# MPEGGroup/mpeg-pcc-tmc2

Measured on AMD Instinct MI355X. Metric: encoder patch+image-gen frames/sec, longdress_vox10 32-frame GOF, higher is better.
Workload: dtype int32/f64

## Files before the change

### mpeg-pcc-tmc2_amd/csrc/api.cpp

```cpp
#include <algorithm>
#include <cstring>
#include <atomic>
#include <chrono>
#include <condition_variable>
#include <cstdarg>
#include <map>
#include <memory>
#include <mutex>

#include "internal.h"

extern char** environ;

namespace tmc2 {
int allowLargeLds( const void* kernel, size_t bytes, int device, size_t staticBytes ) {
  static std::mutex                                 lock;
  static std::map<std::pair<const void*, int>, int> granted;
  std::lock_guard<std::mutex>                       g( lock );
  int& have = granted[{kernel, device}];
  if ( int( bytes ) <= have ) return TMC2_OK;
  const int want = 160 * 1024 - int( ( staticBytes + 63 ) & ~size_t( 63 ) );
  if ( int( bytes ) > want ) {
    setError( "%zu bytes of dynamic LDS requested (+ %zu static): more than a gfx950 workgroup has", bytes, staticBytes );
    return TMC2_E_INVALID;
  }
  TMC2_HIP( hipFuncSetAttribute( kernel, hipFuncAttributeMaxDynamicSharedMemorySize, want ) );
  have = want;
  return TMC2_OK;
}
}

namespace tmc2 {

static thread_local std::string g_lastError;

void setError( const char* fmt, ... ) {
  char    buf[1024];
  va_list ap;
  va_start( ap, fmt );
  vsnprintf( buf, sizeof( buf ), fmt, ap );
  va_end( ap );
  g_lastError = buf;
}

}
struct tmc2_host_gate {
  std::mutex              lock;
  std::condition_variable freed;
  int                     limit = 0, busy = 0;
};
namespace tmc2 {
static std::shared_ptr<tmc2_host_gate> defaultGate() {
  static std::shared_ptr<tmc2_host_gate> g = std::make_shared<tmc2_host_gate>();
  return g;
}
void setHostParallelism( int n ) {
  const auto                  g = defaultGate();
  std::lock_guard<std::mutex> lk( g->lock );
  g->limit = n < 0 ? 0 : n;
  g->freed.notify_all();
}
HostGate::HostGate( const tmc2_ctx* ctx, bool wait ) {
  {
    std::shared_ptr<tmc2_host_gate> own;
    if ( ctx ) {
      std::lock_guard<std::mutex> lk( ctx->optionsLock );
      own = ctx->hostGate;
    }
    gate = own ? own : defaultGate();
  }
  std::unique_lock<std::mutex> lk( gate->lock );
  if ( !wait && gate->limit != 0 && gate->busy >= gate->limit ) return;
  gate->freed.wait( lk, [this] { return gate->limit == 0 || gate->busy < gate->limit; } );
  ++gate->busy;
  held = true;
}
HostGate::~HostGate() { release(); }
void HostGate::release() {
  if ( !held ) return;
  held = false;
  std::lock_guard<std::mutex> g( gate->lock );
  --gate->busy;
  gate->freed.notify_one();
}

static thread_local tmc2_ctx* g_tlsCtx = nullptr;
DevicePool* currentPool() { return g_tlsCtx ? &g_tlsCtx->pool : nullptr; }
ApiScope::ApiScope( tmc2_ctx* ctx ) : prev( g_tlsCtx ) {
  g_tlsCtx = ctx;
  if ( ctx ) (void)hipSetDevice( ctx->device );
}
ApiScope::~ApiScope() { g_tlsCtx = prev; }

int DevicePool::acquire( size_t bytes, void** out, size_t* got ) {
  if ( bytes > ( size_t( 1 ) << 40 ) ) {
    setError( "device allocation of %zu bytes refused", bytes );
    return TMC2_E_INVALID;
  }
  const size_t cls = sizeClass( bytes );
  {
    std::lock_guard<std::mutex> g( lock );
    auto                        it = freeBlocks.find( cls );
    if ( it != freeBlocks.end() && !it->second.empty() ) {
      *out = it->second.back();
      it->second.pop_back();
      *got = cls;
      return TMC2_OK;
    }
  }
  {
    std::lock_guard<std::mutex> g( lock );
    for ( Slab& sl : slabs ) {
      if ( sl.size - sl.used >= cls ) {
        *out = sl.base + sl.used;
        *got = cls;
        sl.used += cls;
        ++carved;
        return TMC2_OK;
      }
    }
  }
  void*      p  = nullptr;
  const auto t0 = std::chrono::steady_clock::now();
  TMC2_HIP( hipMalloc( &p, cls ) );
  const auto t1 = std::chrono::steady_clock::now();
  {
    std::lock_guard<std::mutex> g( lock );
    bytesHeld += cls;
    ++mallocCalls;
    mallocMs += std::chrono::duration<double, std::milli>( t1 - t0 ).count();
  }
  *out = p;
  *got = cls;
  return TMC2_OK;
}
int DevicePool::reserve( size_t bytes ) {
  bytes = ( bytes + 255 ) & ~size_t( 255 );
  void* p = nullptr;
  TMC2_HIP( hipMalloc( &p, bytes ) );
  std::lock_guard<std::mutex> g( lock );
  slabs.push_back( Slab{static_cast<char*>( p ), bytes, 0} );
  bytesHeld += bytes;
  return TMC2_OK;
}
void DevicePool::recycle( void* p, size_t cls ) {
  std::lock_guard<std::mutex> g( lock );
  freeBlocks[cls].push_back( p );
}
void DevicePool::drain() {
  std::lock_guard<std::mutex> g( lock );
  const auto inSlab = [&]( const void* p ) {
    for ( const Slab& sl : slabs )
      if ( static_cast<const char*>( p ) >= sl.base && static_cast<const char*>( p ) < sl.base + sl.size ) return true;
    return false;
  };
  for ( auto& kv : freeBlocks )
    for ( void* p : kv.second )
      if ( !inSlab( p ) ) (void)hipFree( p );
  freeBlocks.clear();
  for ( const Slab& sl : slabs ) (void)hipFree( sl.base );
  slabs.clear();
}

void orientNormalsSpanningTree( const int16_t* xyz, size_t n, const uint32_t* knn, int k, double* normals, void* scratch );

}

using namespace tmc2;

int tmc2_ctx::stageBegin( const char* name ) {
  int id = -1;
  for ( size_t i = 0; i < stages.size(); ++i )
    if ( stages[i].name == name ) id = int( i );
  if ( id < 0 ) {
    StageTimer t;
    t.name = name;
    stages.push_back( t );
    id = int( stages.size() ) - 1;
  }
  stages[id].calls++;
  if ( !timing ) return id;
  hipEvent_t e0 = nullptr, e1 = nullptr;
  if ( freeEvents.size() >= 2 ) {
    e0 = freeEvents.back();
    freeEvents.pop_back();
    e1 = freeEvents.back();
    freeEvents.pop_back();
  } else {
    (void)hipEventCreate( &e0 );
    (void)hipEventCreate( &e1 );
  }
  (void)hipEventRecord( e0, stream );
  stages[id].pending.emplace_back( e0, e1 );
  return id;
}
void tmc2_ctx::stageEnd( int id ) {
  if ( id < 0 || !timing || stages[id].pending.empty() ) return;
  (void)hipEventRecord( stages[id].pending.back().second, stream );
}
void tmc2_ctx::foldStage( StageTimer& t ) {
  for ( auto& pr : t.pending ) {
    float ms = 0.f;
    if ( hipEventSynchronize( pr.second ) == hipSuccess && hipEventElapsedTime( &ms, pr.first, pr.second ) == hipSuccess )
      t.ms += ms;
    freeEvents.push_back( pr.first );
    freeEvents.push_back( pr.second );
  }
  t.pending.clear();
}
void tmc2_ctx::stageAddHostMs( const char* name, double ms ) {
  for ( auto& s : stages )
    if ( s.name == name ) {
      s.ms += ms;
      s.calls++;
      return;
    }
  StageTimer t;
  t.name  = name;
  t.ms    = ms;
  t.calls = 1;
  stages.push_back( t );
}

extern "C" {

const char* tmc2_last_error( void ) { return g_lastError.c_str(); }

int tmc2_ctx_create( int device, tmc2_ctx** out ) {
  if ( !out ) return TMC2_E_INVALID;
  *out      = nullptr;
  int count = 0;
  if ( hipGetDeviceCount( &count ) != hipSuccess || count <= 0 ) {
    setError( "no HIP device visible: this library has no CPU path" );
    return TMC2_E_NO_DEVICE;
  }
  if ( device < 0 || device >= count ) {
    setError( "device %d out of range (%d visible)", device, count );
    return TMC2_E_INVALID;
  }
  TMC2_HIP( hipSetDevice( device ) );
  tmc2_ctx* c = new tmc2_ctx();
  c->device   = device;
  hipDeviceProp_t prop;
  if ( hipGetDeviceProperties( &prop, device ) == hipSuccess ) c->cuCount = prop.multiProcessorCount;
  for ( char** e = environ; e && *e; ++e ) {
    if ( strncmp( *e, "TMC2_", 5 ) != 0 ) continue;
    const char* eq = strchr( *e, '=' );
    if ( !eq ) continue;
    c->options[std::string( *e + 5, size_t( eq - ( *e + 5 ) ) )] = std::string( eq + 1 );
  }
  if ( hipStreamCreateWithFlags( &c->stream, hipStreamNonBlocking ) != hipSuccess ) {
    setError( "hipStreamCreate failed" );
    delete c;
    return TMC2_E_HIP;
  }
  if ( hipHostMalloc( reinterpret_cast<void**>( &c->mailbox ), tmc2_ctx::kMailboxWords * 4, hipHostMallocDefault ) != hipSuccess ) {
    setError( "hipHostMalloc failed (the context's mailbox)" );
    (void)hipStreamDestroy( c->stream );
    delete c;
    return TMC2_E_HIP;
  }
  memset( c->mailbox, 0, tmc2_ctx::kMailboxWords * 4 );
  *out = c;
  return TMC2_OK;
}

int tmc2_ctx_set_option( tmc2_ctx* ctx, const char* key, const char* value ) {
  if ( !ctx || !key || !*key ) {
    tmc2::setError( "tmc2_ctx_set_option: invalid argument" );
    return TMC2_E_INVALID;
  }
  const std::string k = strncmp( key, "TMC2_", 5 ) == 0 ? key + 5 : key;
  std::lock_guard<std::mutex> g( ctx->optionsLock );
  if ( value )
    ctx->options[k] = value;
  else
    ctx->options.erase( k );
  return TMC2_OK;
}
const char* tmc2_ctx_get_option( tmc2_ctx* ctx, const char* key ) {
  if ( !ctx || !key ) return nullptr;
  const auto v = tmc2::ctxOption( ctx, strncmp( key, "TMC2_", 5 ) == 0 ? key + 5 : key );
  if ( !v ) return nullptr;
  static thread_local std::string held;
  held = *v;
  return held.c_str();
}

int tmc2_ctx_reserve( tmc2_ctx* ctx, uint64_t maxPoints, int voxelDimRefine, int bits3d, int maxCanvasWidth, int maxCanvasHeight ) {
  if ( !ctx || maxPoints == 0 || maxPoints > ( uint64_t( 1 ) << 32 ) || bits3d < 1 || bits3d > 16 || maxCanvasWidth < 0 || maxCanvasHeight < 0 ) {
    tmc2::setError( "tmc2_ctx_reserve: invalid argument" );
    return TMC2_E_INVALID;
  }
  tmc2::ApiScope scope( ctx );
  const uint64_t perPoint = voxelDimRefine > 0 && voxelDimRefine <= 2 ? 5500 : 2400;
  const int      gridShift = std::max( 1, bits3d - 1 - ( voxelDimRefine >= 4 ? 2 : ( voxelDimRefine >= 2 ? 1 : 0 ) ) );
  const uint64_t dense     = ( uint64_t( 1 ) << std::min( 33, 3 * gridShift + 1 ) ) / 32 * 8;
  const uint64_t bytes     = maxPoints * perPoint + uint64_t( maxCanvasWidth ) * uint64_t( maxCanvasHeight ) * 64 + dense + ( uint64_t( 64 ) << 20 );
  if ( !ctx->hostC.get<uint32_t>( 4 + ( size_t( maxPoints ) + 4 ) / 4 + 4 ) || !ctx->hostA.get<tmc2::OrientClusterRec>( 64 * 1024 ) ||
       !ctx->hostE.get<tmc2::OrientCompactEdge>( 384 * 1024 ) ) {
    tmc2::setError( "tmc2_ctx_reserve: hipHostMalloc failed" );
    return TMC2_E_HIP;
  }
  return ctx->pool.reserve( size_t( bytes ) );
}
int tmc2_ctx_pool_stats( tmc2_ctx* ctx, uint64_t* bytesHeld, uint64_t* mallocCalls, double* mallocMs, uint64_t* carvedBlocks ) {
  if ( !ctx ) return TMC2_E_INVALID;
  std::lock_guard<std::mutex> g( ctx->pool.lock );
  if ( bytesHeld ) *bytesHeld = ctx->pool.bytesHeld;
  if ( mallocCalls ) *mallocCalls = ctx->pool.mallocCalls;
  if ( mallocMs ) *mallocMs = ctx->pool.mallocMs;
  if ( carvedBlocks ) *carvedBlocks = ctx->pool.carved;
  return TMC2_OK;
}

int tmc2_ctx_device_alloc( tmc2_ctx* ctx, size_t bytes, void** out ) {
  if ( !ctx || !out ) return TMC2_E_INVALID;
  tmc2::ApiScope scope( ctx );
  *out = nullptr;
  TMC2_HIP( hipMalloc( out, std::max<size_t>( bytes, 1 ) ) );
  return TMC2_OK;
}
int tmc2_ctx_device_free( tmc2_ctx* ctx, void* p ) {
  if ( !ctx ) return TMC2_E_INVALID;
  tmc2::ApiScope scope( ctx );
  if ( p ) TMC2_HIP( hipFree( p ) );
  return TMC2_OK;
}
int tmc2_ctx_upload( tmc2_ctx* ctx, void* deviceDst, const void* hostSrc, size_t bytes ) {
  if ( !ctx || ( bytes && ( !deviceDst || !hostSrc ) ) ) return TMC2_E_INVALID;
  tmc2::ApiScope scope( ctx );
  if ( bytes ) TMC2_HIP( hipMemcpyAsync( deviceDst, hostSrc, bytes, hipMemcpyHostToDevice, ctx->stream ) );
  return TMC2_OK;
}
int tmc2_ctx_download( tmc2_ctx* ctx, void* hostDst, const void* deviceSrc, size_t bytes ) {
  if ( !ctx || ( bytes && ( !hostDst || !deviceSrc ) ) ) return TMC2_E_INVALID;
  tmc2::ApiScope scope( ctx );
  if ( bytes ) TMC2_HIP( hipMemcpyAsync( hostDst, deviceSrc, bytes, hipMemcpyDeviceToHost, ctx->stream ) );
  TMC2_HIP( hipStreamSynchronize( ctx->stream ) );
  return TMC2_OK;
}
void* tmc2_ctx_stream( tmc2_ctx* ctx ) { return ctx ? static_cast<void*>( ctx->stream ) : nullptr; }
int   tmc2_ctx_device( tmc2_ctx* ctx ) { return ctx ? ctx->device : -1; }
int   tmc2_ctx_make_current( tmc2_ctx* ctx ) {
  if ( !ctx ) return TMC2_E_INVALID;
  TMC2_HIP( hipSetDevice( ctx->device ) );
  return TMC2_OK;
}

void tmc2_ctx_destroy( tmc2_ctx* ctx ) {
  if ( !ctx ) return;
  ctx->destroyRequested.store( true );
  if ( ctx->liveFrames.load() > 0 ) return;
  if ( ctx->destroyClaimed.exchange( true ) ) return;
  tmc2::destroyContextNow( ctx );
}
}

void tmc2::destroyContextNow( tmc2_ctx* ctx ) {
  (void)hipSetDevice( ctx->device );
  for ( auto& s : ctx->stages ) ctx->foldStage( s );
  for ( auto e : ctx->freeEvents ) (void)hipEventDestroy( e );
  {
    ApiScope scope( ctx );
    ctx->gridBits.release();
    ctx->scanState.release();
    ctx->voxelBitmap.release();
    ctx->constTables.clear();
    ctx->retiredTables.clear();
  }
  if ( ctx->stream ) (void)hipStreamSynchronize( ctx->stream );
  ctx->pool.drain();
  if ( ctx->stream ) (void)hipStreamDestroy( ctx->stream );
  if ( ctx->mailbox ) (void)hipHostFree( ctx->mailbox );
  delete ctx;
}

extern "C" {

int tmc2_host_alloc( size_t bytes, void** out ) {
  if ( !out || bytes == 0 ) return TMC2_E_INVALID;
  *out = nullptr;
  if ( hipHostMalloc( out, bytes, hipHostMallocPortable ) != hipSuccess ) {
    (void)hipGetLastError();
    setError( "host_alloc: %zu bytes of page-locked memory refused", bytes );
    return TMC2_E_HIP;
  }
  return TMC2_OK;
}
void tmc2_host_free( void* p ) {
  if ( p ) (void)hipHostFree( p );
}
int tmc2_host_register( void* p, size_t bytes ) {
  if ( !p || bytes == 0 ) return TMC2_E_INVALID;
  if ( hipHostRegister( p, bytes, hipHostRegisterPortable ) != hipSuccess ) {
    (void)hipGetLastError();
    setError( "host_register: %zu bytes at %p could not be page-locked", bytes, p );
    return TMC2_E_HIP;
  }
  return TMC2_OK;
}
int tmc2_host_unregister( void* p ) {
  if ( !p ) return TMC2_E_INVALID;
  if ( hipHostUnregister( p ) != hipSuccess ) {
    (void)hipGetLastError();
    return TMC2_E_HIP;
  }
  return TMC2_OK;
}

void tmc2_set_host_parallelism( int maxConcurrentHostSteps ) { tmc2::setHostParallelism( maxConcurrentHostSteps ); }
namespace {
std::mutex                                                  g_gatesLock;
std::map<tmc2_host_gate*, std::shared_ptr<tmc2_host_gate>> g_gates;
}
int tmc2_host_gate_create( int maxConcurrentHostSteps, tmc2_host_gate** out ) {
  if ( !out || maxConcurrentHostSteps < 0 ) {
    tmc2::setError( "tmc2_host_gate_create: invalid argument" );
    return TMC2_E_INVALID;
  }
  auto g   = std::make_shared<tmc2_host_gate>();
  g->limit = maxConcurrentHostSteps;
  std::lock_guard<std::mutex> lk( g_gatesLock );
  g_gates[g.get()] = g;
  *out             = g.get();
  return TMC2_OK;
}
void tmc2_host_gate_destroy( tmc2_host_gate* gate ) {
  std::lock_guard<std::mutex> lk( g_gatesLock );
  g_gates.erase( gate );
}
int tmc2_ctx_set_host_gate( tmc2_ctx* ctx, tmc2_host_gate* gate ) {
  if ( !ctx ) {
    tmc2::setError( "tmc2_ctx_set_host_gate: invalid argument" );
    return TMC2_E_INVALID;
  }
  std::shared_ptr<tmc2_host_gate> g;
  if ( gate ) {
    std::lock_guard<std::mutex> lk( g_gatesLock );
    const auto                  it = g_gates.find( gate );
    if ( it == g_gates.end() ) {
      tmc2::setError( "tmc2_ctx_set_host_gate: not a live gate" );
      return TMC2_E_INVALID;
    }
    g = it->second;
  }
  std::lock_guard<std::mutex> lk( ctx->optionsLock );
  ctx->hostGate = g;
  return TMC2_OK;
}

int tmc2_ctx_synchronize( tmc2_ctx* ctx ) {
  if ( !ctx ) return TMC2_E_INVALID;
  TMC2_HIP( hipStreamSynchronize( ctx->stream ) );
  return TMC2_OK;
}

int tmc2_ctx_stage_count( tmc2_ctx* ctx ) { return ctx ? int( ctx->stages.size() ) : 0; }
const char* tmc2_ctx_stage_name( tmc2_ctx* ctx, int i ) {
  return ( ctx && i >= 0 && i < int( ctx->stages.size() ) ) ? ctx->stages[i].name.c_str() : "";
}
double tmc2_ctx_stage_ms( tmc2_ctx* ctx, int i ) {
  if ( !ctx || i < 0 || i >= int( ctx->stages.size() ) ) return 0.0;
  auto& s = ctx->stages[i];
  ctx->foldStage( s );
  return s.ms;
}
void tmc2_ctx_stage_reset( tmc2_ctx* ctx ) {
  if ( !ctx ) return;
  for ( auto& s : ctx->stages ) {
    ctx->foldStage( s );
    s.ms    = 0.0;
    s.calls = 0;
  }
}
long tmc2_ctx_stage_calls( tmc2_ctx* ctx, int i ) {
  return ( ctx && i >= 0 && i < int( ctx->stages.size() ) ) ? ctx->stages[i].calls : 0;
}
void tmc2_ctx_set_timing( tmc2_ctx* ctx, int enabled ) {
  if ( ctx ) ctx->timing = enabled != 0;
}

int tmc2_frame_create( tmc2_ctx* ctx, const int16_t* xyz, const uint8_t* rgb, uint64_t n, tmc2_frame** out ) {
  if ( !ctx || !xyz || !out || n == 0 || n > 0x7FFFFFF0ull ) {
    setError( "frame_create: invalid argument" );
    return TMC2_E_INVALID;
  }
  *out = nullptr;
  ApiScope                    scope( ctx );
  std::unique_ptr<tmc2_frame> f( new tmc2_frame() );
  f->ticket.bind( ctx );
  f->ctx = ctx;
  f->n   = n;
  f->h_xyz.assign( xyz, xyz + 3 * n );
  for ( uint64_t i = 0; i < 3 * n; ++i ) f->geoMax = std::max( f->geoMax, xyz[i] );
  if ( rgb ) f->h_rgb.assign( rgb, rgb + 3 * n );
  std::vector<Pt> pts( n );
  for ( uint64_t i = 0; i < n; ++i ) pts[i] = Pt{xyz[3 * i], xyz[3 * i + 1], xyz[3 * i + 2], 0};
  TMC2_TRY( f->d_pts.alloc( n ) );
  hipStream_t s = ctx->stream;
  TMC2_HIP( hipMemcpyAsync( f->d_pts.p, pts.data(), n * sizeof( Pt ), hipMemcpyHostToDevice, s ) );
  TMC2_HIP( hipStreamSynchronize( s ) );
  if ( rgb ) {
    std::vector<uint8_t> c4( n * 4 );
    for ( uint64_t i = 0; i < n; ++i ) {
      c4[4 * i]     = rgb[3 * i];
      c4[4 * i + 1] = rgb[3 * i + 1];
      c4[4 * i + 2] = rgb[3 * i + 2];
      c4[4 * i + 3] = 0;
    }
    TMC2_TRY( f->d_rgb.alloc( n * 4 ) );
    TMC2_HIP( hipMemcpyAsync( f->d_rgb.p, c4.data(), n * 4, hipMemcpyHostToDevice, s ) );
    TMC2_HIP( hipStreamSynchronize( s ) );
  }
  TMC2_HIP( hipStreamSynchronize( s ) );
  *out = f.release();
  return TMC2_OK;
}

}

namespace tmc2 {
std::optional<std::string> ctxOption( const tmc2_ctx* ctx, const char* key ) {
  if ( !ctx ) {
    const std::string name = std::string( "TMC2_" ) + key;
    const char*       e    = getenv( name.c_str() );
    return e ? std::optional<std::string>( e ) : std::nullopt;
  }
  std::lock_guard<std::mutex> g( ctx->optionsLock );
  const auto                  it = ctx->options.find( key );
  if ( it == ctx->options.end() ) return std::nullopt;
  return it->second;
}
static std::atomic<int> g_refineOverlap{-1};
bool refineOverlap( const tmc2_ctx* ctx ) {
  if ( const auto e = ctxOption( ctx, "REFINE_OVERLAP" ) ) return ( *e )[0] == '1';
  return g_refineOverlap.load( std::memory_order_relaxed ) > 0;
}
static std::atomic<int> g_kdtreeOnHost{-1};
int kdtreePlacement( const tmc2_ctx* ctx ) {
  if ( const auto e = ctxOption( ctx, "KDTREE_HOST" ) )
    if ( ( *e )[0] >= '0' && ( *e )[0] <= '2' ) return ( *e )[0] - '0';
  const int v = g_kdtreeOnHost.load( std::memory_order_relaxed );
  return v < 0 ? 0 : v;
}
int unionPrecheck( const tmc2_ctx* ctx ) {
  const auto e = ctxOption( ctx, "UF_PRECHECK" );
  return e ? ( ( *e )[0] != '0' ) : 1;
}
bool unionAgentScope( const tmc2_ctx* ctx ) {
  const auto e = ctxOption( ctx, "UF_SCOPE" );
  return e && ( *e )[0] == 'a';
}
bool unionCheck( const tmc2_ctx* ctx ) {
  const auto e = ctxOption( ctx, "UF_CHECK" );
  return e && ( *e )[0] == '1';
}
int unionCheckResult( hipStream_t s, const uint32_t* d_bad, const std::string& what ) {
  uint32_t bad[2] = {0, 0};
  TMC2_HIP( hipMemcpyAsync( bad, d_bad, 8, hipMemcpyDeviceToHost, s ) );
  TMC2_HIP( hipStreamSynchronize( s ) );
  if ( bad[0] | bad[1] ) {
    setError( "%s (%u bad links, %u split edges)", what.c_str(), bad[0], bad[1] );
    return TMC2_E_HIP;
  }
  return TMC2_OK;
}
PassOrder passOrder( const tmc2_frame* f, const char* option ) {
  const auto order = ctxOption( f->ctx, option );
  const char o     = order ? ( *order )[0] : 'c';
  const bool tree  = o == 't' && f->haveTree && f->tree.perm.p && f->tree.perm.count >= f->n;
  return {o != 'i', tree ? f->tree.perm.p : nullptr};
}
void setRefineOverlapDefault( int on ) { g_refineOverlap.store( on ? 1 : 0, std::memory_order_relaxed ); }
void setKdtreePlacement( int mode ) { g_kdtreeOnHost.store( mode < 0 || mode > 2 ? 0 : mode, std::memory_order_relaxed ); }
int buildKdTreePlaced( tmc2_ctx* ctx, const Pt* d_pts, uint64_t n, const int16_t* hostXyz, const char* stage, DeviceTree& tree ) {
  const int placement = kdtreePlacement( ctx );
  HostGate gate( ctx, placement == 1 );
  if ( placement == 0 || !gate.held ) {
    StageScope span( ctx, stage );
    return buildKdTreeDevice( ctx, d_pts, n, tree );
  }
  Pt*       hp = ctx->hostD.get<Pt>( n );
  uint32_t* hi = ctx->hostA.get<uint32_t>( n );
  if ( !hp || !hi ) {
    setError( "kdtree: hipHostMalloc failed" );
    return TMC2_E_HIP;
  }
  hipStream_t s = ctx->stream;
  if ( !hostXyz ) {
    TMC2_HIP( hipMemcpyAsync( hp, d_pts, n * sizeof( Pt ), hipMemcpyDeviceToHost, s ) );
    TMC2_HIP( hipStreamSynchronize( s ) );
  }
  KdTreeHost host;
  {
    const auto t0 = std::chrono::steady_clock::now();
    if ( hostXyz )
      for ( uint64_t i = 0; i < n; ++i ) hp[i] = Pt{hostXyz[3 * size_t( i )], hostXyz[3 * size_t( i ) + 1], hostXyz[3 * size_t( i ) + 2], 0};
    host.buildInPlace( hp, hi, n );
    const auto t1 = std::chrono::steady_clock::now();
    ctx->stageAddHostMs( ( std::string( stage ) + "_host" ).c_str(), std::chrono::duration<double, std::milli>( t1 - t0 ).count() );
  }
  gate.release();
  TMC2_TRY( tree.ptsTree.alloc( n ) );
  TMC2_TRY( tree.perm.alloc( n ) );
  TMC2_TRY( tree.nodes.alloc( host.nodes.size() ) );
  TMC2_HIP( hipMemcpyAsync( tree.ptsTree.p, hp, n * sizeof( Pt ), hipMemcpyHostToDevice, s ) );
  TMC2_HIP( hipMemcpyAsync( tree.perm.p, hi, n * sizeof( uint32_t ), hipMemcpyHostToDevice, s ) );
  TMC2_HIP( hipMemcpyAsync( tree.nodes.p, host.nodes.data(), host.nodes.size() * sizeof( KdNode ), hipMemcpyHostToDevice, s ) );
  TMC2_HIP( hipStreamSynchronize( s ) );
  for ( int d = 0; d < 3; ++d ) tree.lo[d] = host.lo[d], tree.hi[d] = host.hi[d];
  tree.depth = host.depth;
  tree.n     = n;
  return TMC2_OK;
}
}

const int* tmc2_ctx::constTable( uint64_t key, const std::vector<int>& host ) {
  auto it = constTables.find( key );
  if ( it != constTables.end() && it->second->host == host ) return it->second->dev.p;
  auto entry = std::make_unique<ConstTable>();
  if ( entry->dev.alloc( std::max<size_t>( host.size(), 1 ) ) != TMC2_OK ) return nullptr;
  entry->host = host;
  if ( !host.empty() && hipMemcpyAsync( entry->dev.p, entry->host.data(), host.size() * sizeof( int ), hipMemcpyHostToDevice, stream ) != hipSuccess ) {
    tmc2::setError( "constTable: upload failed" );
    return nullptr;
  }
  const int* p = entry->dev.p;
  if ( it != constTables.end() ) retiredTables.push_back( std::move( it->second ) );
  constTables[key] = std::move( entry );
  return p;
}

void tmc2_frame::resetDerived() {
  haveTree = haveKnn = haveNormals = havePartition = haveMutual = false;
  havePatches = haveAttr16 = false;
  patchesChanged();
  patches.clear();
  packOrder.clear();
  packMatch.clear();
  depthCount = occCount = 0;
  rounds = packedHeight = packedWidth = 0;
  refineJob.reset();
}

int tmc2::normalsCompute( tmc2_frame* f, int k, int orientation, const std::function<int()>* beforeHostWalk ) {
  TMC2_TRY( tmc2_normals_compute_normals( f, k ) );
  if ( orientation == 0 ) return TMC2_OK;
  if ( orientation != 1 ) {
    setError( "normalOrientation=%d unsupported (0 none, 1 spanning tree)", orientation );
    return TMC2_E_UNSUPPORTED;
  }
  tmc2::ApiScope scope( f->ctx );
  return orientNormalsHost( f, beforeHostWalk );
}

int tmc2_frame::ensureTree() {
  if ( haveTree ) return TMC2_OK;
  TMC2_TRY( tmc2::buildKdTreePlaced( ctx, d_pts.p, n, h_xyz.data(), "kdtree_build", tree ) );
  haveTree = true;
  return TMC2_OK;
}

extern "C" {

int tmc2_kdtree_build( tmc2_frame* f ) {
  if ( !f ) return TMC2_E_INVALID;
  tmc2::ApiScope scope( f->ctx );
  return f->ensureTree();
}

int tmc2_frame_get_kdtree_order( tmc2_frame* f, uint32_t* perm, int32_t* depth ) {
  if ( !f || !perm ) return TMC2_E_INVALID;
  tmc2::ApiScope scope( f->ctx );
  TMC2_TRY( f->ensureTree() );
  TMC2_HIP( hipMemcpyAsync( perm, f->tree.perm.p, f->n * sizeof( uint32_t ), hipMemcpyDeviceToHost, f->ctx->stream ) );
  TMC2_HIP( hipStreamSynchronize( f->ctx->stream ) );
  if ( depth ) *depth = f->tree.depth;
  return TMC2_OK;
}

void tmc2_set_kdtree_placement( int mode ) { tmc2::setKdtreePlacement( mode ); }
void tmc2_set_refine_overlap( int on ) { tmc2::setRefineOverlapDefault( on ); }

void tmc2_frame_destroy( tmc2_frame* f ) {
  if ( !f ) return;
  ApiScope scope( f->ctx );
  (void)hipStreamSynchronize( f->ctx->stream );
  delete f;
}

uint64_t tmc2_frame_point_count( const tmc2_frame* f ) { return f ? f->n : 0; }

int tmc2_frame_reset( tmc2_frame* f ) {
  if ( !f ) return TMC2_E_INVALID;
  tmc2::ApiScope scope( f->ctx );
  f->resetDerived();
  return TMC2_OK;
}

int tmc2_kdtree_search( tmc2_frame* f, const int16_t* queries, uint64_t nq, int k, uint32_t* idx, uint32_t* dist2 ) {
  if ( !f || !queries || !idx || nq == 0 || nq > ( 1ull << 32 ) ) {
    setError( "kdtree_search: invalid argument" );
    return TMC2_E_INVALID;
  }
  if ( k != 1 && k != 4 && k != 8 && k != 16 ) {
    setError( "kdtree_search: k = %d unsupported (1, 4, 8 or 16)", k );
    return TMC2_E_UNSUPPORTED;
  }
  tmc2::ApiScope scope( f->ctx );
  TMC2_TRY( f->ensureTree() );
  std::vector<Pt> q( nq );
  bool bounded = true;
  for ( uint64_t i = 0; i < nq; ++i ) {
    q[i] = Pt{queries[3 * i], queries[3 * i + 1], queries[3 * i + 2], 0};
    for ( int d = 0; d < 3; ++d ) bounded = bounded && queries[3 * i + d] >= -4096 && queries[3 * i + d] <= 12287;
  }
  DevBuf<Pt>       d_q;
  DevBuf<uint32_t> d_idx, d_dist;
  TMC2_TRY( d_q.alloc( nq ) );
  TMC2_TRY( d_idx.alloc( nq * size_t( k ) ) );
  if ( dist2 ) TMC2_TRY( d_dist.alloc( nq * size_t( k ) ) );
  hipStream_t s = f->ctx->stream;
  TMC2_HIP( hipMemcpyAsync( d_q.p, q.data(), nq * sizeof( Pt ), hipMemcpyHostToDevice, s ) );
  TMC2_TRY( launchKnnQueries( f, d_q.p, nq, k, d_idx.p, dist2 ? d_dist.p : nullptr, bounded ) );
  TMC2_HIP( hipMemcpyAsync( idx, d_idx.p, nq * size_t( k ) * 4, hipMemcpyDeviceToHost, s ) );
  if ( dist2 ) TMC2_HIP( hipMemcpyAsync( dist2, d_dist.p, nq * size_t( k ) * 4, hipMemcpyDeviceToHost, s ) );
  TMC2_HIP( hipStreamSynchronize( s ) );
  return TMC2_OK;
}

int tmc2_normals_compute_normals( tmc2_frame* f, int k ) {
  if ( !f ) return TMC2_E_INVALID;
  tmc2::ApiScope scope( f->ctx );
  TMC2_TRY( f->ensureTree() );
  if ( !f->haveKnn || f->k != k ) TMC2_TRY( launchKnnSelf( f, k ) );
  return launchNormals( f );
}

int tmc2_normals_orient( tmc2_frame* f ) {
  if ( !f ) return TMC2_E_INVALID;
  tmc2::ApiScope scope( f->ctx );
  return orientNormalsHost( f );
}

int tmc2_normals_compute( tmc2_frame* f, int k, int orientation ) { return tmc2::normalsCompute( f, k, orientation, nullptr ); }

int tmc2_frame_get_normals( tmc2_frame* f, double* normals ) {
  if ( !f || !normals || !f->haveNormals ) {
    setError( "get_normals: no normals" );
    return TMC2_E_STATE;
  }
  tmc2::ApiScope scope( f->ctx );
  TMC2_HIP( hipMemcpyAsync( normals, f->d_normals.p, f->n * 3 * sizeof( double ), hipMemcpyDeviceToHost, f->ctx->stream ) );
  TMC2_HIP( hipStreamSynchronize( f->ctx->stream ) );
  return TMC2_OK;
}

int tmc2_frame_set_normals( tmc2_frame* f, const double* normals ) {
  if ( !f || !normals ) return TMC2_E_INVALID;
  tmc2::ApiScope scope( f->ctx );
  TMC2_TRY( f->d_normals.alloc( f->n * 3 ) );
  TMC2_HIP( hipMemcpyAsync( f->d_normals.p, normals, f->n * 3 * sizeof( double ), hipMemcpyHostToDevice, f->ctx->stream ) );
  TMC2_HIP( hipStreamSynchronize( f->ctx->stream ) );
  f->haveNormals = true;
  return TMC2_OK;
}

int tmc2_frame_get_adjacency( tmc2_frame* f, uint32_t* adj ) {
  if ( !f || !adj || !f->haveKnn ) {
    setError( "get_adjacency: no adjacency" );
    return TMC2_E_STATE;
  }
  tmc2::ApiScope scope( f->ctx );
  TMC2_HIP( hipMemcpyAsync( adj, f->d_knn.p, f->n * size_t( f->k ) * 4, hipMemcpyDeviceToHost, f->ctx->stream ) );
  TMC2_HIP( hipStreamSynchronize( f->ctx->stream ) );
  return TMC2_OK;
}

int tmc2_weight_normal( tmc2_frame* f, int geometryBitDepth3D, double minWeightEPP, double weight[3] ) {
  if ( !f || !weight ) return TMC2_E_INVALID;
  tmc2::ApiScope scope( f->ctx );
  return weightNormal( f, geometryBitDepth3D, minWeightEPP, weight );
}

int tmc2_segmenter_initial_segmentation( tmc2_frame* f, const double weight[3] ) {
  if ( !f || !weight ) return TMC2_E_INVALID;
  tmc2::ApiScope scope( f->ctx );
  return launchInitialSegmentation( f, weight );
}

int tmc2_segmenter_refine_grid_based( tmc2_frame* f, int maxNNCount, double lambda, int iterationCount, int voxDim,
                                      int searchRadius ) {
  if ( !f ) return TMC2_E_INVALID;
  tmc2::ApiScope scope( f->ctx );
  return refineGridBased( f, maxNNCount, lambda, iterationCount, voxDim, searchRadius );
}

int tmc2_frame_get_partition( tmc2_frame* f, uint32_t* partition ) {
  if ( !f || !partition || !f->havePartition ) {
    setError( "get_partition: no partition" );
    return TMC2_E_STATE;
  }
  tmc2::ApiScope scope( f->ctx );
  std::vector<uint8_t> tmp( f->n );
  TMC2_HIP( hipMemcpyAsync( tmp.data(), f->d_partition.p, f->n, hipMemcpyDeviceToHost, f->ctx->stream ) );
  TMC2_HIP( hipStreamSynchronize( f->ctx->stream ) );
  for ( uint64_t i = 0; i < f->n; ++i ) partition[i] = tmp[i];
  return TMC2_OK;
}

int tmc2_frame_set_partition( tmc2_frame* f, const uint32_t* partition ) {
  if ( !f || !partition ) return TMC2_E_INVALID;
  tmc2::ApiScope scope( f->ctx );
  std::vector<uint8_t> tmp( f->n );
  for ( uint64_t i = 0; i < f->n; ++i ) {
    if ( partition[i] > 5 ) {
      setError( "set_partition: label %u of point %llu out of range (0..5)", partition[i], (unsigned long long)i );
      return TMC2_E_INVALID;
    }
    tmp[i] = uint8_t( partition[i] );
  }
  TMC2_TRY( f->d_partition.alloc( f->n ) );
  TMC2_HIP( hipMemcpyAsync( f->d_partition.p, tmp.data(), f->n, hipMemcpyHostToDevice, f->ctx->stream ) );
  TMC2_HIP( hipStreamSynchronize( f->ctx->stream ) );
  f->havePartition = true;
  return TMC2_OK;
}

int tmc2_host_kdtree_build( const int16_t* xyz, uint64_t n, uint32_t* perm, uint64_t* nodeCount, int32_t* depth ) {
  if ( !xyz || !perm || n == 0 ) return TMC2_E_INVALID;
  KdTreeHost t;
  t.build( xyz, n );
  memcpy( perm, t.perm.data(), n * sizeof( uint32_t ) );
  if ( nodeCount ) *nodeCount = t.nodes.size();
  if ( depth ) *depth = t.depth;
  return TMC2_OK;
}

int tmc2_host_orient_normals( const int16_t* xyz, uint64_t n, const uint32_t* knn, int k, double* normals ) {
  if ( !xyz || !knn || !normals || k < 1 ) return TMC2_E_INVALID;
  orientNormalsSpanningTree( xyz, n, knn, k, normals, nullptr );
  return TMC2_OK;
}

}
```

### mpeg-pcc-tmc2_amd/csrc/internal.h

```cpp
#pragma once
#include <hip/hip_runtime.h>

#include <algorithm>
#include <cstdint>
#include <cstdio>
#include <cstring>
#include <initializer_list>
#include <atomic>
#include <map>
#include <memory>
#include <mutex>
#include <optional>
#include <string>
#include <functional>
#include <vector>

#include "tmc2hip.h"

namespace tmc2 {

void setError( const char* fmt, ... );

#define TMC2_HIP( expr )                                                                        \
  do {                                                                                          \
    hipError_t e_ = ( expr );                                                                   \
    if ( e_ != hipSuccess ) {                                                                   \
      tmc2::setError( "%s:%d: %s -> %s", __FILE__, __LINE__, #expr, hipGetErrorString( e_ ) ); \
      return TMC2_E_HIP;                                                                        \
    }                                                                                           \
  } while ( 0 )

#define TMC2_TRY( expr )          \
  do {                            \
    int r_ = ( expr );            \
    if ( r_ != TMC2_OK ) return r_; \
  } while ( 0 )

struct DevicePool {
  std::mutex                                 lock;
  std::map<size_t, std::vector<void*>>       freeBlocks;
  size_t                                     bytesHeld = 0;
  struct Slab {
    char*  base;
    size_t size, used;
  };
  std::vector<Slab>                          slabs;
  size_t                                     mallocCalls = 0, carved = 0;
  double                                     mallocMs = 0.0;
  int  reserve( size_t bytes );
  static size_t sizeClass( size_t bytes ) {
    size_t c = 256;
    while ( c < bytes ) c <<= 1;
    return c;
  }
  int  acquire( size_t bytes, void** out, size_t* got );
  void recycle( void* p, size_t cls );
  void drain();
};
DevicePool* currentPool();

template <typename T>
struct DevBuf {
  T*          p = nullptr;
  size_t      count = 0;
  size_t      cls   = 0;
  DevicePool* pool  = nullptr;
  DevBuf() = default;
  DevBuf( const DevBuf& ) = delete;
  DevBuf& operator=( const DevBuf& ) = delete;
  ~DevBuf() { release(); }
  void release() {
    if ( p ) {
      if ( pool )
        pool->recycle( p, cls );
      else
        (void)hipFree( p );
    }
    p     = nullptr;
    count = 0;
    pool  = nullptr;
  }
  int alloc( size_t n ) {
    if ( n <= count && p ) return TMC2_OK;
    release();
    if ( n == 0 ) n = 1;
    DevicePool* pl = currentPool();
    if ( pl ) {
      void*  q   = nullptr;
      size_t got = 0;
      if ( n > ( size_t( 1 ) << 40 ) / sizeof( T ) ) {
        setError( "device allocation of %zu elements refused", n );
        return TMC2_E_INVALID;
      }
      TMC2_TRY( pl->acquire( n * sizeof( T ), &q, &got ) );
      p     = reinterpret_cast<T*>( q );
      cls   = got;
      pool  = pl;
      count = got / sizeof( T );
    } else {
      TMC2_HIP( hipMalloc( reinterpret_cast<void**>( &p ), n * sizeof( T ) ) );
      count = n;
    }
    return TMC2_OK;
  }
  size_t bytes() const { return count * sizeof( T ); }
};

struct alignas( 16 ) KdNode {
  int32_t a;
  int32_t b;
  int16_t divlow;
  int16_t divhigh;
  int32_t dim;
};

struct alignas( 8 ) Pt {
  int16_t x, y, z, w;
};
struct KdTreeHost {
  std::vector<uint32_t> perm;
  std::vector<Pt>       ptsTree;
  std::vector<KdNode>   nodes;
  int32_t               lo[3], hi[3];
  int                   depth = 0;
  void                  build( const int16_t* xyz, size_t n );
  void                  buildInPlace( Pt* pts, uint32_t* ind, size_t n );
};


#if defined( __HIP_DEVICE_COMPILE__ ) && !defined( __gfx950__ ) && !defined( __gfx942__ )
#error "loadStaleOk: the stale-view argument is written for the gfx942 / gfx950 cache hierarchy"
#endif
#if defined( __HIPCC__ )
template <typename T>
__device__ __forceinline__ T loadStaleOk( const T* p, bool agent = false ) {
  return agent ? __hip_atomic_load( p, __ATOMIC_RELAXED, __HIP_MEMORY_SCOPE_AGENT )
               : __hip_atomic_load( p, __ATOMIC_RELAXED, __HIP_MEMORY_SCOPE_WORKGROUP );
}
#endif

constexpr uint32_t chunkedGrid( uint32_t blocks ) { return ( blocks + 7u ) & ~7u; }
#if defined( __HIPCC__ )
struct XcdPlace {
  uint32_t xcd, perXcd, slot;
};
__device__ __forceinline__ XcdPlace xcdPlace() { return {blockIdx.x & 7u, gridDim.x >> 3, blockIdx.x >> 3}; }
__device__ __forceinline__ uint32_t chunkedBlock( uint32_t perXcd ) {
  const XcdPlace at = xcdPlace();
  return at.xcd * perXcd + at.slot;
}
__device__ __forceinline__ uint32_t logicalBlock( bool chunked ) { return chunked ? chunkedBlock( xcdPlace().perXcd ) : blockIdx.x; }
__device__ __forceinline__ uint32_t chunkedIndex() { return logicalBlock( !( gridDim.x & 7u ) ) * blockDim.x + threadIdx.x; }
__device__ __forceinline__ uint32_t pointOfLane( const uint32_t* __restrict__ perm, bool chunked, uint32_t n ) {
  const uint32_t at = logicalBlock( chunked ) * blockDim.x + threadIdx.x;
  return at < n ? ( perm ? perm[at] : at ) : n;
}
#endif

constexpr int kMaxCanvasDim = 32767;
__host__ __device__ __forceinline__ uint32_t packPixel( int x, int y, int layer, bool hasD1 ) {
  return uint32_t( x ) | ( uint32_t( y ) << 15 ) | ( uint32_t( layer ) << 30 ) | ( hasD1 ? 1u << 31 : 0u );
}
__host__ __device__ __forceinline__ uint32_t pixelX( uint32_t p ) { return p & 0x7FFFu; }
__host__ __device__ __forceinline__ uint32_t pixelY( uint32_t p ) { return ( p >> 15 ) & 0x7FFFu; }
__host__ __device__ __forceinline__ uint32_t pixelLayer( uint32_t p ) { return ( p >> 30 ) & 1u; }
__host__ __device__ __forceinline__ bool     pixelHasD1( uint32_t p ) { return ( p >> 31 ) != 0u; }

struct PlaceDev {
  int32_t u0, v0, orient;
  int32_t sizeU, sizeV, sizeU0, sizeV0;
  int32_t tileBase;
  int32_t u1, v1, d1;
  int32_t axN, axT, axB, mode;
  int32_t pad;
  int64_t depthOff;
};

struct TreeDev {
  const Pt*       ptsTree = nullptr;
  const uint32_t* perm    = nullptr;
  const KdNode*   nodes   = nullptr;
  int32_t         lo[3] = {0, 0, 0}, hi[3] = {0, 0, 0};
  int             depth = 0;
  uint64_t        n     = 0;
  bool            queriesBounded = false;
  bool            queriesTight   = false;
};
enum class QueryBox { Any, Bounded, Tight };

struct DeviceTree {
  DevBuf<Pt>       ptsTree;
  DevBuf<uint32_t> perm;
  DevBuf<KdNode>   nodes;
  int32_t          lo[3] = {0, 0, 0}, hi[3] = {0, 0, 0};
  int              depth = 0;
  uint64_t         n     = 0;
  TreeDev          view( QueryBox queries ) const {
    TreeDev t;
    t.ptsTree = ptsTree.p, t.perm = perm.p, t.nodes = nodes.p;
    for ( int d = 0; d < 3; ++d ) t.lo[d] = lo[d], t.hi[d] = hi[d];
    t.depth          = depth;
    t.n              = n;
    t.queriesBounded = queries != QueryBox::Any;
    t.queriesTight   = queries == QueryBox::Tight;
    return t;
  }
};

struct StageTimer {
  std::string                                    name;
  std::vector<std::pair<hipEvent_t, hipEvent_t>> pending;
  double                                         ms    = 0.0;
  long                                           calls = 0;
};

}

namespace tmc2 {
struct PinnedBuf {
  void*  p     = nullptr;
  size_t bytes = 0;
  PinnedBuf() = default;
  PinnedBuf( const PinnedBuf& ) = delete;
  PinnedBuf& operator=( const PinnedBuf& ) = delete;
  ~PinnedBuf() {
    if ( p ) (void)hipHostFree( p );
  }
  template <typename T>
  T* get( size_t count ) {
    const size_t need = count * sizeof( T );
    if ( need > bytes ) {
      if ( p ) (void)hipHostFree( p );
      p     = nullptr;
      bytes = 0;
      const size_t cap = need + need / 4;
      if ( hipHostMalloc( &p, cap, hipHostMallocDefault ) != hipSuccess ) {
        p = nullptr;
        return nullptr;
      }
      bytes = cap;
    }
    return reinterpret_cast<T*>( p );
  }
};
struct StageScope;
struct RefineJob;
}

struct tmc2_ctx {
  std::atomic<int>              liveFrames{0};
  std::atomic<bool>             destroyRequested{false}, destroyClaimed{false};
  int                           device = 0;
  tmc2::DevicePool              pool;
  tmc2::PinnedBuf               hostA, hostB, hostC, hostD, hostE;
  tmc2::PinnedBuf               hostTables, hostRecords;
  std::vector<int32_t>          orientScratch;
  tmc2::DevBuf<uint2>           gridBits;
  int                           refineCapTier = 0;
  uint32_t                      refineHitsPerVoxel = 640;
  tmc2::DevBuf<unsigned long long> scanState;
  uint32_t                      scanEpoch = 0, scanTickets = 0;
  tmc2::DevBuf<uint32_t>        voxelBitmap;
  std::map<uint32_t, int>       kdLevelHint;
  struct ConstTable {
    tmc2::DevBuf<int> dev;
    std::vector<int>  host;
  };
  std::map<uint64_t, std::unique_ptr<ConstTable>> constTables;
  std::vector<std::unique_ptr<ConstTable>>        retiredTables;
  const int* constTable( uint64_t key, const std::vector<int>& host );
  uint32_t* mailbox = nullptr;
  static constexpr size_t kMailboxWords = 1024;
  volatile uint32_t* answerLine( int line ) const { return mailbox + size_t( line ) * 16; }
  enum { kAnswerRefineVoxels = 1, kAnswerPatchRound = 2, kAnswerRecon = 3, kAnswerOrientHead = 4, kAnswerTreeDepth = 5, kAnswerGeoError = 6, kAnswerAttrError = 7, kAnswerTreeLevels = 8  };
  std::map<std::string, std::string> options;
  mutable std::mutex                 optionsLock;
  std::shared_ptr<tmc2_host_gate>    hostGate;
  hipStream_t                   stream = nullptr;
  std::vector<tmc2::StageTimer> stages;
  std::vector<hipEvent_t>       freeEvents;
  bool                          timing = true;
  int                           cuCount = 256;
  void foldStage( tmc2::StageTimer& t );
  void stageAddHostMs( const char* name, double ms );

 private:
  friend struct tmc2::StageScope;
  int  stageBegin( const char* name );
  void stageEnd( int id );
};

namespace tmc2 {
struct StageScope {
  StageScope( tmc2_ctx* c, const char* name ) : ctx( c ), id( c->stageBegin( name ) ) {}
  StageScope( const StageScope& ) = delete;
  StageScope& operator=( const StageScope& ) = delete;
  ~StageScope() { end(); }
  void end() { ctx->stageEnd( id ), id = -1; }

 private:
  tmc2_ctx* ctx;
  int       id;
};
void destroyContextNow( tmc2_ctx* ctx );
struct FrameTicket {
  tmc2_ctx* ctx = nullptr;
  void      bind( tmc2_ctx* c ) {
    ctx = c;
    c->liveFrames.fetch_add( 1 );
  }
  ~FrameTicket() {
    if ( ctx && ctx->liveFrames.fetch_sub( 1 ) == 1 && ctx->destroyRequested.load() && !ctx->destroyClaimed.exchange( true ) )
      destroyContextNow( ctx );
  }
};
}

struct tmc2_frame {
  tmc2::FrameTicket ticket;
  tmc2_ctx* ctx = nullptr;
  uint64_t  n   = 0;
  int       k   = 0;
  std::vector<int16_t> h_xyz;
  std::vector<uint8_t> h_rgb;
  bool                 haveTree = false;
  int                  ensureTree();
  std::shared_ptr<tmc2::RefineJob> refineJob;
  void resetDerived();
  void patchesChanged() { havePacking = false, packingChanged(); }
  void packingChanged() { haveGeometryImages = false, canvasesChanged(); }
  void canvasesChanged() {
    haveAttributeImages = haveReconstruction = false;
    haveBoundaryTypes = haveColors16 = haveSmoothed = haveRgbPost = false;
  }
  tmc2::DevBuf<tmc2::Pt>     d_pts;
  tmc2::DeviceTree           tree;
  tmc2::DevBuf<uint8_t>      d_rgb;
  tmc2::DevBuf<uint32_t>     d_knn;
  tmc2::DevBuf<double>       d_normals;
  tmc2::DevBuf<uint8_t>      d_partition;
  bool haveKnn = false, haveNormals = false, havePartition = false;
  tmc2::DevBuf<uint16_t>     d_mutual;
  bool haveMutual = false;
  int16_t geoMax = 0;
  std::vector<tmc2_patch> patches;
  tmc2::DevBuf<int16_t>   d_depth0, d_depth1;
  tmc2::DevBuf<uint8_t>   d_occupancy;
  int64_t                 depthCount = 0, occCount = 0;
  int                     rounds     = 0;
  std::vector<int32_t>    packMatch;
  bool                    havePatches = false;
  int                     growPools();
  std::vector<int32_t>    packOrder;
  int                     packedHeight = 0, packedWidth = 0;
  bool                    havePacking = false, haveGeometryImages = false;
  int                     canvasW = 0, canvasH = 0, occPrecision = 0;
  tmc2::DevBuf<uint8_t>   d_occMap;
  tmc2::DevBuf<uint8_t>   d_occVideo;
  tmc2::DevBuf<uint32_t>  d_blockToPatch;
  tmc2::DevBuf<uint16_t>  d_geo;
  tmc2::DevBuf<tmc2::PlaceDev> d_place;
  tmc2::DevBuf<uint32_t>  d_tilePatch;
  uint32_t                tileCount = 0;
  uint64_t                reconCount = 0;
  bool                    haveAttributeImages = false, haveReconstruction = false;
  tmc2::DevBuf<tmc2::Pt>  d_recon;
  tmc2::DevBuf<uint32_t>  d_pointToPixel;
  tmc2::DevBuf<uint8_t>   d_reconRgb;
  tmc2::DevBuf<uint8_t>   d_attr;
  tmc2::DevBuf<uint8_t>   d_boundaryType;
  tmc2::DevBuf<uint64_t>  d_colors16;
  tmc2::DevBuf<tmc2::Pt>  d_reconSmoothed;
  tmc2::DevBuf<uint8_t>   d_rgbPost;
  tmc2::DevBuf<uint16_t>  d_attr16;
  bool                    haveAttr16 = false;
  bool                    haveBoundaryTypes = false, haveColors16 = false, haveSmoothed = false, haveRgbPost = false;
  tmc2::DeviceTree        reconTree;
  int                     geometryBitDepth3D = 0;
};

namespace tmc2 {
struct HostGate {
  explicit HostGate( const tmc2_ctx* ctx, bool wait = true );
  ~HostGate();
  void release();
  bool held = false;
  std::shared_ptr<tmc2_host_gate> gate;
};
void setHostParallelism( int n );
struct ApiScope {
  tmc2_ctx* prev;
  explicit ApiScope( tmc2_ctx* ctx );
  ~ApiScope();
};
int launchKnnSelf( tmc2_frame* f, int k );
int launchKnnQueries( tmc2_frame* f, const Pt* d_queries, uint64_t nq, int k, uint32_t* d_idx, uint32_t* d_dist,
                      bool queriesBounded );
int launchKnnTree( tmc2_ctx* ctx, const TreeDev& tree, const Pt* d_queries, uint64_t nq, int k, uint32_t* d_idx,
                   uint32_t* d_dist, const char* stage );
int launchKnnSplit( tmc2_ctx* ctx, const TreeDev& tree, const Pt* d_queries, uint64_t nq, int k, uint32_t* d_easy, uint32_t* d_idx,
                    uint32_t* d_dist, const char* stage, bool uniqueTreeRows = false );
int generateAttributeImages( tmc2_frame* f );
int reconstructPointCloud( tmc2_frame* f );
int uploadPlacement( tmc2_frame* f );
int launchNormals( tmc2_frame* f );
int orientNormalsHost( tmc2_frame* f, const std::function<int()>* beforeHostWalk = nullptr );
int normalsCompute( tmc2_frame* f, int k, int orientation, const std::function<int()>* beforeHostWalk );
int ensureMutualMask( tmc2_frame* f );
int launchEdgeDots( tmc2_frame* f, double* d_edgeDot );
constexpr size_t kOrientNegCountWords = 64 * 32;
int launchApplyOrientation( tmc2_frame* f, const int8_t* d_sign, uint32_t* d_negCount );
struct OrientCrossEdge {
  uint32_t u, v;
  double   d;
};
struct OrientCompactEdge {
  uint32_t u, v, c2, pad;
  double   d;
};
struct OrientClusterRec {
  uint32_t off;
  uint32_t seedPoint;
  uint32_t seedParity;
};
struct OrientCompact {
  uint32_t                 clusters;
  const OrientClusterRec*  rec;
  const OrientCompactEdge* edges;
};
bool orientCompactSigns( const OrientCompact& g, double tau, int8_t* clusterSign, uint32_t* component, std::vector<uint32_t>& seeds,
                         std::vector<uint32_t>& seedClusters );
void resolveSeedSignsCompact( const OrientCompact& g, int kNN, const std::vector<uint32_t>& seeds, const std::vector<uint32_t>& seedClusters,
                              const uint32_t* component, const uint32_t* who, const double* normals, const int16_t* xyz0, int8_t* clusterSign );
int gatherSeedTables( tmc2_frame* f, const uint32_t* d_cid, const uint8_t* d_parity, const std::vector<uint32_t>& seeds,
                      std::vector<uint32_t>& who, std::vector<double>& normals );
int orientSpanningTreeSigns( const int16_t* xyz, size_t n, const uint32_t* knn, int k, const double* normals,
                             const double* edgeDot, int8_t* sign, void* scratch, bool tryContraction, const tmc2_ctx* ctx );
double orientFirstTau( const tmc2_ctx* ctx );
int contractOrientationDevice( tmc2_frame* f, double tau, DevBuf<uint32_t>& d_cid,
                               DevBuf<uint8_t>& d_parity, OrientCompact& g, bool& ok );
int launchClusterSigns( tmc2_frame* f, const uint32_t* d_cid, const uint8_t* d_parity, const int8_t* d_clusterSign,
                        int8_t* d_sign );
int launchInitialSegmentation( tmc2_frame* f, const double weight[3] );
int weightNormal( tmc2_frame* f, int bits, double minWeightEPP, double w[3] );
int segmentPatches( tmc2_frame* f, const tmc2_segmenter_params* sp );
int packFlexibleHost( tmc2_frame* f, int presetWidth, int occRes, int numTilesHor, double tileHeightToWidthRatio );
struct GpaFrameIO {
  std::vector<tmc2_patch> list;
  std::vector<uint8_t>    occ;
  std::vector<int32_t>    match;
  int                     width = 0, height = 0;
};
int globalPatchAllocationCore( std::vector<GpaFrameIO>& frames, int minW, int minH, int occRes );
int installPacking( tmc2_frame* f, const GpaFrameIO& g );
int generateGeometryImages( tmc2_frame* f, int W, int H, int occRes, int occPrecision );
int rgb444ToYuv420Device( tmc2_ctx* ctx, const uint8_t* d_rgb, int W, int H, int filter, uint8_t* d_yuv );
int yuv420ToYuv444Device( tmc2_ctx* ctx, const uint8_t* d_yuv, int W, int H, int filter, uint16_t* d_out );
int refineGridBased( tmc2_frame* f, int maxNNCount, double lambda, int iterationCount, int voxDim, int searchRadius );
void setRefineOverlapDefault( int on );
inline int refineBallCells( int r2 ) {
  int R = 0, ball = 0;
  while ( R * R < r2 ) ++R;
  for ( int dz = -R; dz <= R; ++dz )
    for ( int dy = -R; dy <= R; ++dy )
      for ( int dx = -R; dx <= R; ++dx ) ball += dx * dx + dy * dy + dz * dz < r2;
  return ball;
}
inline bool refineBallFits( int r2 ) { return r2 >= 1 && r2 <= 128 && refineBallCells( r2 ) <= 4096 - 160; }
bool refineOverlap( const tmc2_ctx* ctx );
int refinePrepareGeometry( tmc2_frame* f, int maxNNCount, double lambda, int iterationCount, int voxDim, int searchRadius );
inline uint32_t cappedBlocks( const tmc2_ctx* ctx, size_t wanted ) {
  return uint32_t( std::max<size_t>( 1, std::min<size_t>( wanted, size_t( 8 ) * size_t( ctx->cuCount ) ) ) );
}
std::optional<std::string> ctxOption( const tmc2_ctx* ctx, const char* key );
int  kdtreePlacement( const tmc2_ctx* ctx );
int  unionPrecheck( const tmc2_ctx* ctx );
bool unionCheck( const tmc2_ctx* ctx );
bool unionAgentScope( const tmc2_ctx* ctx );
int unionCheckResult( hipStream_t s, const uint32_t* d_bad, const std::string& what );
struct PassOrder {
  bool            chunked;
  const uint32_t* perm;
};
PassOrder passOrder( const tmc2_frame* f, const char* option );
int buildKdTreeDevice( tmc2_ctx* ctx, const Pt* d_pts, uint64_t n, DeviceTree& tree );
int buildKdTreePlaced( tmc2_ctx* ctx, const Pt* d_pts, uint64_t n, const int16_t* hostXyz, const char* stage, DeviceTree& tree );
int allowLargeLds( const void* kernel, size_t bytes, int device, size_t staticBytes = 64 );
struct ScanAnswer {
  volatile uint32_t* host       = nullptr;
  const uint32_t*    carry      = nullptr;
  int                carryWords = 0;
};
int exclusiveScanU32( tmc2_ctx* ctx, const uint32_t* d_in, uint32_t* d_out, size_t n, uint32_t* d_total, ScanAnswer answer = ScanAnswer() );
struct FillRegion {
  void*   p;
  size_t  bytes;
  uint8_t value;
};
int fillRegions( tmc2_ctx* ctx, std::initializer_list<FillRegion> regions );
}
```

### mpeg-pcc-tmc2_amd/csrc/kdtree_device.hip

```cpp
#include <algorithm>
#include <cstring>

#include "internal.h"

namespace tmc2 {
namespace {

constexpr uint32_t kNone      = 0xFFFFFFFFu;
constexpr int      kBlock     = 256;
constexpr int      kWaves     = kBlock / 64;
constexpr int      kScanTile  = kBlock * 8;
constexpr int      kLeafMax   = 10;
constexpr int      kMaxLevels = 64;

struct BuildSeg {
  uint32_t begin, end;
  uint32_t node, parent;
  int32_t  mn[3], mx[3];
  int16_t  lo[3], hi[3];
  uint8_t  side, pdim;
  uint8_t  split, cutDim;
  int32_t  cut;
  uint32_t mid;
  uint32_t slot;
};

struct RetiredSeg {
  uint32_t begin, end, node, level;
  int16_t  lo[3], hi[3];
  int32_t  root;
};

struct HugeSeg {
  uint32_t begin, end, node, level;
  int16_t  lo[3], hi[3];
  int32_t  root;
  int32_t  mn[3], mx[3];
};

struct BuildArgs {
  const Pt* pts;
  uint32_t  n, tiles;
  Pt*       P;
  uint32_t *perm, *seg;
  BuildSeg *segA, *segB;
  KdNode*   nodes;
  uint32_t *loc1, *loc2, *tile1, *tile2;
  uint32_t* counts;
  uint32_t* nodeCount;
  int32_t*  rootBox;
  uint32_t* levels;
  RetiredSeg* retired;
  uint32_t*   retiredCount;
  uint32_t*   bigCount;
  HugeSeg*    huge;
  uint32_t*   hugeCount;
  uint32_t    hugeMax;
  uint32_t    retireMax, splitMax;
  struct LvSeg *lvA, *lvB;
  uint16_t*   list;
  struct LvPartial* partial;
  unsigned long long* pieceProfile;
  uint32_t    decideRng;
  uint32_t*   finishDepth;
  uint32_t*   ticket;
  volatile uint32_t* hostSmall;
  volatile uint32_t* hostDepth;
};

__device__ __forceinline__ int coordOf( const Pt p, int d ) { return d == 0 ? p.x : ( d == 1 ? p.y : p.z ); }

struct SplitRule {
  int     dim;
  int32_t cut;
};
__device__ __forceinline__ SplitRule splitOf( const int16_t ( &lo )[3], const int16_t ( &hi )[3], const int32_t ( &mn )[3],
                                              const int32_t ( &mx )[3] ) {
  const int32_t maxSpan = max( int32_t( hi[0] ) - lo[0], max( int32_t( hi[1] ) - lo[1], int32_t( hi[2] ) - lo[2] ) );
  SplitRule     r;
  r.dim              = 0;
  int32_t bestSpread = -1;
#pragma unroll
  for ( int d = 0; d < 3; ++d ) {
    if ( double( int32_t( hi[d] ) - lo[d] ) > ( 1.0 - 0.00001 ) * double( maxSpan ) ) {
      const int32_t spread = mx[d] - mn[d];
      if ( spread > bestSpread ) {
        bestSpread = spread;
        r.dim      = d;
      }
    }
  }
  const int32_t l = r.dim == 0 ? lo[0] : ( r.dim == 1 ? lo[1] : lo[2] ), h = r.dim == 0 ? hi[0] : ( r.dim == 1 ? hi[1] : hi[2] );
  const int32_t a = r.dim == 0 ? mn[0] : ( r.dim == 1 ? mn[1] : mn[2] ), b = r.dim == 0 ? mx[0] : ( r.dim == 1 ? mx[1] : mx[2] );
  r.cut           = min( max( ( l + h ) / 2, a ), b );
  return r;
}

constexpr int      kHugeWaves = 16;
constexpr uint32_t kHugeLimit = 131072;
constexpr int      kHugeNodes = 2 * int( kHugeLimit / 4096 ) + 4;
struct HugeNode {
  uint32_t begin, end;
  uint32_t node;
  int16_t  lo[3], hi[3];
  int16_t  mn[3], mx[3];
  uint16_t depth;
};

__device__ __forceinline__ uint32_t blockClassLists( const Pt* pts, uint32_t count, int dim, int32_t c, uint32_t* listGE,
                                                     uint32_t* listLT, uint32_t* waveCnt ) {
  const int lane = threadIdx.x & 63, wave = threadIdx.x >> 6;
  uint32_t  mGE = 0, mIn = 0;
  int       buf = 0;
  for ( uint32_t base = 0; base < count; base += 4u * blockDim.x, buf ^= 1 ) {
    const uint32_t i0 = base + 4u * threadIdx.x;
    bool           ge[4];
    uint32_t       cGE = 0, cIn = 0;
#pragma unroll
    for ( int j = 0; j < 4; ++j ) {
      const bool    in = i0 + j < count;
      const int32_t x  = coordOf( pts[in ? i0 + j : 0u], dim );
      ge[j]            = in && x >= c;
      cGE += uint32_t( ge[j] ), cIn += uint32_t( in );
    }
    uint32_t inc = cGE | ( cIn << 16 );
#pragma unroll
    for ( int off = 1; off < 64; off <<= 1 ) {
      const uint32_t t = __shfl_up( inc, off, 64 );
      if ( lane >= off ) inc += t;
    }
    if ( lane == 63 ) waveCnt[buf * kHugeWaves + wave] = inc;
    __syncthreads();
    uint32_t before = 0, total = 0;
#pragma unroll
    for ( int w = 0; w < kHugeWaves; ++w ) {
      const uint32_t cw = waveCnt[buf * kHugeWaves + w];
      total += cw;
      before += w < wave ? cw : 0u;
    }
    before += inc - ( cGE | ( cIn << 16 ) );
    uint32_t atGE = mGE + ( before & 0xFFFFu ) + 0u, atIn = mIn + ( before >> 16 );
#pragma unroll
    for ( int j = 0; j < 4; ++j ) {
      if ( i0 + j < count ) {
        if ( ge[j] )
          listGE[atGE] = i0 + j;
        else
          listLT[atIn - atGE] = i0 + j;
        atGE += uint32_t( ge[j] ), ++atIn;
      }
    }
    mGE += total & 0xFFFFu, mIn += total >> 16;
  }
  return mGE;
}

__device__ __forceinline__ uint32_t blockSweep( Pt* pts, uint32_t* id, uint32_t count, int dim, int32_t c, uint32_t* listGE,
                                                uint32_t* listLT, uint32_t* waveCnt ) {
  const uint32_t nGE = blockClassLists( pts, count, dim, c, listGE, listLT, waveCnt ), nL = count - nGE;
  __syncthreads();
  for ( uint32_t t = threadIdx.x; t < min( nGE, nL ); t += blockDim.x ) {
    const uint32_t x = listGE[t];
    if ( x >= nL ) break;
    const uint32_t y  = listLT[nL - 1u - t];
    const Pt       px = pts[x], py = pts[y];
    const uint32_t ix = id[x], iy = id[y];
    pts[x] = py, pts[y] = px, id[x] = iy, id[y] = ix;
  }
  __syncthreads();
  return nL;
}

__global__ __launch_bounds__( 64 * kHugeWaves ) void hugeSegmentsKernel( BuildArgs a ) {
  __shared__ HugeNode sNode[2][kHugeNodes];
  __shared__ uint32_t sCount[2], waveCnt[2 * kHugeWaves];
  __shared__ int32_t  red[kHugeWaves][12];
  const int      lane = threadIdx.x & 63, wave = threadIdx.x >> 6;
  const uint32_t total = *a.hugeCount;
  for ( uint32_t s = blockIdx.x; s < total; s += gridDim.x ) {
    const HugeSeg seg = a.huge[s];
    __syncthreads();
    if ( threadIdx.x == 0 ) {
      HugeNode r;
      r.begin = 0, r.end = seg.end - seg.begin, r.node = seg.node, r.depth = 0;
      for ( int d = 0; d < 3; ++d ) r.lo[d] = seg.lo[d], r.hi[d] = seg.hi[d], r.mn[d] = int16_t( seg.mn[d] ), r.mx[d] = int16_t( seg.mx[d] );
      sNode[0][0] = r;
      sCount[0] = 1, sCount[1] = 0;
    }
    __syncthreads();
    int cur = 0;
    for ( uint32_t depth = 0;; ++depth ) {
      const uint32_t nCur = sCount[cur];
      if ( nCur == 0 ) break;
      for ( uint32_t t = 0; t < nCur; ++t ) {
        const HugeNode q     = sNode[cur][t];
        const uint32_t count = q.end - q.begin;
        if ( uint32_t( q.depth ) + seg.level >= uint32_t( kMaxLevels ) - 2u ) {
          if ( threadIdx.x == 0 ) atomicMax( a.finishDepth, 0x10000u );
          continue;
        }
        Pt*       pts = a.P + seg.begin + q.begin;
        uint32_t* id  = a.perm + seg.begin + q.begin;
        int32_t   mn[3], mx[3];
        const bool isRoot = seg.root != 0 && depth == 0;
        int16_t    lo[3], hi[3];
        for ( int d = 0; d < 3; ++d ) mn[d] = q.mn[d], mx[d] = q.mx[d], lo[d] = isRoot ? q.mn[d] : q.lo[d], hi[d] = isRoot ? q.mx[d] : q.hi[d];
        const SplitRule rule  = splitOf( lo, hi, mn, mx );
        uint32_t*       listA = a.loc1 + seg.begin + q.begin;
        uint32_t*       listB = a.loc2 + seg.begin + q.begin;
        const uint32_t  lt    = blockSweep( pts, id, count, rule.dim, rule.cut, listA, listB, waveCnt );
        const uint32_t  le    = lt + blockSweep( pts + lt, id + lt, count - lt, rule.dim, rule.cut + 1, listA, listB, waveCnt );
        const uint32_t  half  = count / 2;
        const uint32_t  idx   = lt > half ? lt : ( le < half ? le : half );
        int32_t r[12];
#pragma unroll
        for ( int k = 0; k < 12; ++k ) r[k] = ( k % 6 ) < 3 ? 0x7FFFFFFF : int32_t( 0x80000000 );
        for ( uint32_t base = 0; base < count; base += 4u * blockDim.x ) {
          Pt p[4];
#pragma unroll
          for ( int j = 0; j < 4; ++j ) {
            const uint32_t i = base + j * blockDim.x + threadIdx.x;
            p[j]             = pts[i < count ? i : 0u];
          }
#pragma unroll
          for ( int j = 0; j < 4; ++j ) {
            const uint32_t i = base + j * blockDim.x + threadIdx.x;
            if ( i < count ) {
              const int o = i < idx ? 0 : 6;
              if ( o == 0 ) {
                r[0] = min( r[0], int32_t( p[j].x ) ), r[1] = min( r[1], int32_t( p[j].y ) ), r[2] = min( r[2], int32_t( p[j].z ) );
                r[3] = max( r[3], int32_t( p[j].x ) ), r[4] = max( r[4], int32_t( p[j].y ) ), r[5] = max( r[5], int32_t( p[j].z ) );
              } else {
                r[6] = min( r[6], int32_t( p[j].x ) ), r[7] = min( r[7], int32_t( p[j].y ) ), r[8] = min( r[8], int32_t( p[j].z ) );
                r[9] = max( r[9], int32_t( p[j].x ) ), r[10] = max( r[10], int32_t( p[j].y ) ), r[11] = max( r[11], int32_t( p[j].z ) );
              }
            }
          }
        }
#pragma unroll
        for ( int off = 32; off > 0; off >>= 1 )
#pragma unroll
          for ( int k = 0; k < 12; ++k ) {
            const int32_t o = __shfl_xor( r[k], off, 64 );
            r[k]            = ( k % 6 ) < 3 ? min( r[k], o ) : max( r[k], o );
          }
        if ( lane == 0 )
          for ( int k = 0; k < 12; ++k ) red[wave][k] = r[k];
        __syncthreads();
        if ( threadIdx.x == 0 ) {
          for ( int w = 0; w < kHugeWaves; ++w )
            for ( int k = 0; k < 12; ++k ) r[k] = ( k % 6 ) < 3 ? min( r[k], red[w][k] ) : max( r[k], red[w][k] );
          const uint32_t id0 = atomicAdd( a.nodeCount, 2u );
          KdNode         nd;
          nd.a = int32_t( id0 ), nd.b = int32_t( id0 + 1 ), nd.divlow = int16_t( r[3 + rule.dim] ), nd.divhigh = int16_t( r[6 + rule.dim] ),
          nd.dim = rule.dim;
          a.nodes[q.node] = nd;
          HugeNode child[2];
          child[0].begin = q.begin, child[0].end = q.begin + idx, child[0].node = id0;
          child[1].begin = q.begin + idx, child[1].end = q.end, child[1].node = id0 + 1;
          for ( int c = 0; c < 2; ++c ) {
            child[c].depth = uint16_t( q.depth + 1 );
            for ( int d = 0; d < 3; ++d )
              child[c].lo[d] = lo[d], child[c].hi[d] = hi[d], child[c].mn[d] = int16_t( r[6 * c + d] ), child[c].mx[d] = int16_t( r[6 * c + 3 + d] );
          }
          const int16_t cut = int16_t( rule.cut );
          if ( rule.dim == 0 ) child[0].hi[0] = cut, child[1].lo[0] = cut;
          if ( rule.dim == 1 ) child[0].hi[1] = cut, child[1].lo[1] = cut;
          if ( rule.dim == 2 ) child[0].hi[2] = cut, child[1].lo[2] = cut;
          for ( int c = 0; c < 2; ++c ) {
            const uint32_t cc = child[c].end - child[c].begin, level = seg.level + child[c].depth;
            if ( cc <= uint32_t( kLeafMax ) ) {
              KdNode leaf;
              leaf.a = int32_t( seg.begin + child[c].begin ), leaf.b = int32_t( seg.begin + child[c].end ), leaf.divlow = leaf.divhigh = 0,
              leaf.dim = -1;
              a.nodes[child[c].node] = leaf;
              atomicMax( a.finishDepth, level + 1u );
            } else if ( cc <= a.retireMax ) {
              RetiredSeg rs;
              rs.begin = seg.begin + child[c].begin, rs.end = seg.begin + child[c].end, rs.node = child[c].node, rs.level = level, rs.root = 0;
              for ( int d = 0; d < 3; ++d ) rs.lo[d] = child[c].lo[d], rs.hi[d] = child[c].hi[d];
              a.retired[atomicAdd( a.retiredCount, 1u )] = rs;
            } else {
              sNode[cur ^ 1][sCount[cur ^ 1]++] = child[c];
            }
          }
        }
        __syncthreads();
      }
      if ( threadIdx.x == 0 ) sCount[cur] = 0;
      cur ^= 1;
      __syncthreads();
    }
  }
}

constexpr int      kPieceMax  = 4096;
constexpr int      kPieceRecs = kPieceMax / ( kLeafMax + 1 ) + 2;
constexpr uint16_t kNoRec     = 0xFFFFu;
constexpr uint32_t kNoKey     = 0xFFFFFFFFu;

struct alignas( 8 ) PieceRec {
  uint16_t begin, end;
  int16_t  cut;
  uint8_t  dim, unused0;
  uint16_t edge1, rb1;
  uint16_t edge2, rb2;
  uint16_t mid;
  uint16_t child[2];
  uint16_t unused1;
  uint32_t node;
  int32_t  lmax, rmin;
  int16_t  lo[3], hi[3];
  int32_t  mn[3], mx[3];
};
static_assert( sizeof( PieceRec ) == 72, "PieceRec layout" );
struct PieceHot0 {
  uint32_t be, dc;
};
struct PieceHot1 {
  uint32_t e1rb1, e2rb2;
};
struct PieceHot2 {
  uint32_t midc0, c1;
};

__device__ __forceinline__ void pieceBarrier() { asm volatile( "s_waitcnt lgkmcnt(0)\n\ts_barrier" ::: "memory" ); }

typedef short pkShort2 __attribute__( ( ext_vector_type( 2 ) ) );
__device__ __forceinline__ uint32_t pkMin( uint32_t a, uint32_t b ) {
  return __builtin_bit_cast( uint32_t, __builtin_elementwise_min( __builtin_bit_cast( pkShort2, a ), __builtin_bit_cast( pkShort2, b ) ) );
}
__device__ __forceinline__ uint32_t pkMax( uint32_t a, uint32_t b ) {
  return __builtin_bit_cast( uint32_t, __builtin_elementwise_max( __builtin_bit_cast( pkShort2, a ), __builtin_bit_cast( pkShort2, b ) ) );
}
__device__ __forceinline__ uint32_t pk2( int lo16, int hi16 ) { return ( uint32_t( lo16 ) & 0xFFFFu ) | ( uint32_t( hi16 ) << 16 ); }
__device__ __forceinline__ int      pkLo( uint32_t v ) { return int( int16_t( v & 0xFFFFu ) ); }
__device__ __forceinline__ int      pkHi( uint32_t v ) { return int( int16_t( v >> 16 ) ); }

template <int WAVES>
__device__ __forceinline__ uint32_t pieceScan( uint32_t v, uint32_t* waveTot ) {
  const int lane = threadIdx.x & 63, wave = threadIdx.x >> 6;
  uint32_t  inc  = v;
#pragma unroll
  for ( int off = 1; off < 64; off <<= 1 ) {
    const uint32_t t = __shfl_up( inc, off, 64 );
    if ( lane >= off ) inc += t;
  }
  if ( lane == 63 ) waveTot[wave] = inc;
  pieceBarrier();
  uint32_t before = 0;
#pragma unroll
  for ( int w = 0; w < WAVES; w += 4 ) {
    const uint4 t = *reinterpret_cast<const uint4*>( waveTot + w );
    before += ( w + 0 < wave ? t.x : 0u ) + ( w + 1 < wave ? t.y : 0u ) + ( w + 2 < wave ? t.z : 0u ) + ( w + 3 < wave ? t.w : 0u );
  }
  return before + inc - v;
}

__device__ __forceinline__ bool waveSegMinMaxPacked( uint32_t key, uint32_t& A, uint32_t& B, uint32_t& C, int lane ) {
#pragma unroll
  for ( int off = 1; off < 64; off <<= 1 ) {
    const uint32_t ok = __shfl_down( key, off, 64 );
    const uint32_t oa = __shfl_down( A, off, 64 ), ob = __shfl_down( B, off, 64 ), oc = __shfl_down( C, off, 64 );
    if ( lane + off < 64 && ok == key ) A = pkMin( A, oa ), B = pkMax( B, ob ), C = pkMin( C, oc );
  }
  const uint32_t pk = __shfl_up( key, 1, 64 );
  return key != kNoKey && ( lane == 0 || pk != key );
}

__device__ __forceinline__ void ldsMin( int32_t* slot, int32_t v ) {
  if ( v < *reinterpret_cast<volatile int32_t*>( slot ) ) atomicMin( slot, v );
}
__device__ __forceinline__ void ldsMax( int32_t* slot, int32_t v ) {
  if ( v > *reinterpret_cast<volatile int32_t*>( slot ) ) atomicMax( slot, v );
}


struct LvSeg {
  uint32_t begin, end;
  uint32_t cutInfo;
  uint32_t edge1;
  uint32_t slot;
  uint32_t childNode;
  uint32_t node, parent;
  int16_t  lo[3], hi[3];
  uint8_t  side, pdim;
  uint16_t unused;
  int32_t  mn[3], mx[3];
};

constexpr int kLandBlock = 256;
constexpr int kLandRounds = 2;
struct LvPartial {
  uint32_t slot;
  uint32_t v[6];
  uint32_t unused;
};

__device__ __forceinline__ void lvReport( LvSeg* child, int mnx, int mny, int mnz, int mxx, int mxy, int mxz ) {
  if ( mnx < loadStaleOk( &child->mn[0] ) ) atomicMin( &child->mn[0], mnx );
  if ( mny < loadStaleOk( &child->mn[1] ) ) atomicMin( &child->mn[1], mny );
  if ( mnz < loadStaleOk( &child->mn[2] ) ) atomicMin( &child->mn[2], mnz );
  if ( mxx > loadStaleOk( &child->mx[0] ) ) atomicMax( &child->mx[0], mxx );
  if ( mxy > loadStaleOk( &child->mx[1] ) ) atomicMax( &child->mx[1], mxy );
  if ( mxz > loadStaleOk( &child->mx[2] ) ) atomicMax( &child->mx[2], mxz );
}

__device__ __forceinline__ uint32_t lvPrefix( const uint32_t* __restrict__ loc, const uint32_t* sums, uint32_t tiles, uint32_t i, uint32_t n ) {
  return i < n ? loc[i] + sums[i / kScanTile] : sums[tiles];
}

__device__ __forceinline__ uint32_t lvPartner( const uint16_t* __restrict__ list, const uint32_t* sums, uint32_t from, uint32_t to, uint32_t G ) {
  uint32_t lo = from / kScanTile, hi = ( to - 1u ) / kScanTile;
  while ( lo < hi ) {
    const uint32_t mid = ( lo + hi + 1u ) / 2u;
    if ( mid * kScanTile - sums[mid] <= G )
      lo = mid;
    else
      hi = mid - 1u;
  }
  return lo * kScanTile + list[size_t( lo ) * kScanTile + ( G - ( lo * kScanTile - sums[lo] ) )];
}

__global__ __launch_bounds__( kBlock ) void lvInitKernel( BuildArgs a ) {
  __shared__ int blockRange[6 * kWaves];
  const uint32_t n = a.n, gsize = gridDim.x * blockDim.x;
  const int      lane = threadIdx.x & 63, wave = threadIdx.x >> 6;
  int mnx = 0x7FFFFFFF, mny = mnx, mnz = mnx, mxx = int( 0x80000000 ), mxy = mxx, mxz = mxx;
  for ( uint32_t i = blockIdx.x * blockDim.x + threadIdx.x; i < n; i += gsize ) {
    const Pt p = a.pts[i];
    a.P[i]     = p;
    a.perm[i]  = i;
    a.seg[i]   = 0;
    mnx = min( mnx, int( p.x ) ), mny = min( mny, int( p.y ) ), mnz = min( mnz, int( p.z ) );
    mxx = max( mxx, int( p.x ) ), mxy = max( mxy, int( p.y ) ), mxz = max( mxz, int( p.z ) );
  }
#pragma unroll
  for ( int off = 32; off > 0; off >>= 1 ) {
    mnx = min( mnx, __shfl_xor( mnx, off, 64 ) ), mny = min( mny, __shfl_xor( mny, off, 64 ) ), mnz = min( mnz, __shfl_xor( mnz, off, 64 ) );
    mxx = max( mxx, __shfl_xor( mxx, off, 64 ) ), mxy = max( mxy, __shfl_xor( mxy, off, 64 ) ), mxz = max( mxz, __shfl_xor( mxz, off, 64 ) );
  }
  if ( lane == 0 ) {
    int* w = blockRange + 6 * wave;
    w[0] = mnx, w[1] = mny, w[2] = mnz, w[3] = mxx, w[4] = mxy, w[5] = mxz;
  }
  __syncthreads();
  if ( threadIdx.x < 6 ) {
    int v = blockRange[threadIdx.x];
    for ( int w = 1; w < kWaves; ++w ) v = threadIdx.x < 3 ? min( v, blockRange[6 * w + threadIdx.x] ) : max( v, blockRange[6 * w + threadIdx.x] );
    int32_t* slot = threadIdx.x < 3 ? &a.lvA[0].mn[threadIdx.x] : &a.lvA[0].mx[threadIdx.x - 3];
    if ( threadIdx.x < 3 ) {
      if ( v < loadStaleOk( slot ) ) atomicMin( slot, v );
    } else {
      if ( v > loadStaleOk( slot ) ) atomicMax( slot, v );
    }
  }
}
__global__ void lvRootKernel( BuildArgs a ) {
  if ( threadIdx.x < kMaxLevels + 16 ) a.counts[threadIdx.x] = 0;
  __syncthreads();
  if ( threadIdx.x != 0 ) return;
  LvSeg r{};
  r.begin = 0, r.end = a.n, r.node = 0, r.parent = kNone;
  for ( int d = 0; d < 3; ++d ) r.mn[d] = 0x7FFFFFFF, r.mx[d] = int32_t( 0x80000000 );
  a.lvA[0]     = r;
  a.counts[0]  = 1;
  *a.nodeCount = 1;
}

constexpr int kDecideThreads = 1024;
constexpr int kDecideRng     = 2000;
__global__ __launch_bounds__( kDecideThreads ) void lvDecideKernel( BuildArgs a, uint32_t level ) {
  __shared__ uint32_t waveTot[kDecideThreads / 64];
  __shared__ uint32_t sCarry;
  __shared__ int32_t  sRng[kDecideRng][6];
  LvSeg*         cur   = ( level & 1 ) ? a.lvB : a.lvA;
  const uint32_t count = a.counts[level], nodeBase = *a.nodeCount;
  const int      lane = threadIdx.x & 63, wave = threadIdx.x >> 6;
  if ( threadIdx.x == 0 ) sCarry = 0;
  const bool inLds = level > 0 && count <= a.decideRng;
  if ( inLds ) {
    for ( uint32_t t = threadIdx.x; t < count * 6u; t += kDecideThreads ) sRng[t / 6u][t % 6u] = ( t % 6u ) < 3u ? 0x7FFFFFFF : int32_t( 0x80000000 );
    __syncthreads();
  }
  if ( level > 0 ) {
    const uint32_t nPart = ( a.n + uint32_t( kLandBlock * kLandRounds ) - 1u ) / uint32_t( kLandBlock * kLandRounds );
    for ( uint32_t base = 0; base < nPart; base += kDecideThreads ) {
      const uint32_t t = base + threadIdx.x;
      LvPartial      pt;
      pt.slot = kNone;
      if ( t < nPart ) pt = a.partial[t];
#pragma unroll
      for ( int c = 0; c < 2; ++c ) {
        uint32_t A = pt.v[3 * c], B = pt.v[3 * c + 1], C = pt.v[3 * c + 2];
        if ( waveSegMinMaxPacked( pt.slot == kNone ? kNoKey : pt.slot, A, B, C, lane ) ) {
          if ( inLds ) {
            int32_t* r = sRng[pt.slot + c];
            ldsMin( &r[0], pkLo( A ) ), ldsMin( &r[1], pkHi( A ) ), ldsMin( &r[2], pkLo( C ) );
            ldsMax( &r[3], pkLo( B ) ), ldsMax( &r[4], pkHi( B ) ), ldsMax( &r[5], ~pkHi( C ) );
          } else {
            lvReport( cur + pt.slot + c, pkLo( A ), pkHi( A ), pkLo( C ), pkLo( B ), pkHi( B ), ~pkHi( C ) );
          }
        }
      }
    }
    if ( !inLds ) asm volatile( "s_waitcnt vmcnt(0)" ::: "memory" );
  }
  __syncthreads();
  for ( uint32_t base = 0; base < count; base += kDecideThreads ) {
    const uint32_t s     = base + threadIdx.x;
    uint32_t       split = 0;
    LvSeg*         q     = cur + s;
    if ( s < count ) {
      const bool root = q->parent == kNone;
      int32_t    mn[3], mx[3], lo[3], hi[3];
#pragma unroll
      for ( int d = 0; d < 3; ++d ) {
        mn[d] = __hip_atomic_load( &q->mn[d], __ATOMIC_RELAXED, __HIP_MEMORY_SCOPE_AGENT );
        mx[d] = __hip_atomic_load( &q->mx[d], __ATOMIC_RELAXED, __HIP_MEMORY_SCOPE_AGENT );
        if ( inLds ) mn[d] = min( mn[d], sRng[s][d] ), mx[d] = max( mx[d], sRng[s][3 + d] );
        lo[d] = root ? mn[d] : int32_t( q->lo[d] );
        hi[d] = root ? mx[d] : int32_t( q->hi[d] );
      }
      if ( root ) {
        for ( int d = 0; d < 3; ++d ) a.rootBox[d] = mn[d], a.rootBox[3 + d] = mx[d];
      } else {
        const int pd = q->pdim;
        if ( q->side == 0 )
          a.nodes[q->parent].divlow = int16_t( pd == 0 ? mx[0] : ( pd == 1 ? mx[1] : mx[2] ) );
        else
          a.nodes[q->parent].divhigh = int16_t( pd == 0 ? mn[0] : ( pd == 1 ? mn[1] : mn[2] ) );
      }
      const uint32_t cnt = q->end - q->begin;
      if ( cnt <= uint32_t( kLeafMax ) ) {
        KdNode nd;
        nd.a = int32_t( q->begin ), nd.b = int32_t( q->end ), nd.divlow = nd.divhigh = 0, nd.dim = -1;
        a.nodes[q->node] = nd;
      } else if ( cnt <= a.retireMax ) {
        RetiredSeg r;
        r.begin = q->begin, r.end = q->end, r.node = q->node, r.level = level;
        r.root  = root ? 1 : 0;
        for ( int d = 0; d < 3; ++d ) r.lo[d] = q->lo[d], r.hi[d] = q->hi[d];
        a.retired[atomicAdd( a.retiredCount, 1u )] = r;
      } else if ( cnt <= a.hugeMax ) {
        HugeSeg r;
        r.begin = q->begin, r.end = q->end, r.node = q->node, r.level = level;
        r.root  = root ? 1 : 0;
        for ( int d = 0; d < 3; ++d ) r.lo[d] = q->lo[d], r.hi[d] = q->hi[d], r.mn[d] = mn[d], r.mx[d] = mx[d];
        a.huge[atomicAdd( a.hugeCount, 1u )] = r;
      } else {
        const int32_t maxSpan = max( hi[0] - lo[0], max( hi[1] - lo[1], hi[2] - lo[2] ) );
        const double  limit   = ( 1.0 - 0.00001 ) * double( maxSpan );
        int           dim     = 0;
        int32_t       best    = -1;
        if ( double( hi[0] - lo[0] ) > limit && mx[0] - mn[0] > best ) best = mx[0] - mn[0], dim = 0;
        if ( double( hi[1] - lo[1] ) > limit && mx[1] - mn[1] > best ) best = mx[1] - mn[1], dim = 1;
        if ( double( hi[2] - lo[2] ) > limit && mx[2] - mn[2] > best ) best = mx[2] - mn[2], dim = 2;
        const int32_t l = dim == 0 ? lo[0] : ( dim == 1 ? lo[1] : lo[2] ), h = dim == 0 ? hi[0] : ( dim == 1 ? hi[1] : hi[2] );
        const int32_t lowest = dim == 0 ? mn[0] : ( dim == 1 ? mn[1] : mn[2] ), highest = dim == 0 ? mx[0] : ( dim == 1 ? mx[1] : mx[2] );
        const int32_t cut = min( max( ( l + h ) / 2, lowest ), highest );
        q->cutInfo = ( uint32_t( cut ) & 0xFFFFu ) | ( uint32_t( dim ) << 16 ) | ( 1u << 24 );
        if ( root )
          for ( int d = 0; d < 3; ++d ) q->lo[d] = int16_t( mn[d] ), q->hi[d] = int16_t( mx[d] );
        split = 1;
      }
      if ( !split ) q->cutInfo = 0;
    }
    uint32_t inc = split;
#pragma unroll
    for ( int off = 1; off < 64; off <<= 1 ) {
      const uint32_t t = __shfl_up( inc, off, 64 );
      if ( lane >= off ) inc += t;
    }
    if ( lane == 63 ) waveTot[wave] = inc;
    __syncthreads();
    uint32_t before = sCarry, all = 0;
    for ( int w = 0; w < kDecideThreads / 64; ++w ) {
      all += waveTot[w];
      before += w < wave ? waveTot[w] : 0u;
    }
    const uint32_t rank = before + inc - split;
    if ( split ) q->slot = 2u * rank, q->childNode = nodeBase + 2u * rank;
    __syncthreads();
    if ( threadIdx.x == 0 ) sCarry += all;
    __syncthreads();
  }
  if ( threadIdx.x == 0 ) {
    a.counts[level + 1] = 2u * sCarry;
    *a.nodeCount        = nodeBase + 2u * sCarry;
  }
  if ( a.hostSmall ) {
    if ( threadIdx.x == 0 ) __threadfence();
    __syncthreads();
    if ( threadIdx.x < kMaxLevels + 16 ) a.hostSmall[threadIdx.x] = __hip_atomic_load( &a.counts[threadIdx.x], __ATOMIC_RELAXED, __HIP_MEMORY_SCOPE_AGENT );
  }
}

template <bool FIRST>
__global__ __launch_bounds__( kBlock ) void lvFlagKernel( BuildArgs a, uint32_t level ) {
  __shared__ uint32_t waveSum[kWaves];
  const uint32_t n = a.n, tiles = a.tiles;
  const int      lane = threadIdx.x & 63, wave = threadIdx.x >> 6;
  LvSeg*         cur   = ( level & 1 ) ? a.lvB : a.lvA;
  LvSeg*         next  = ( level & 1 ) ? a.lvA : a.lvB;
  const uint32_t count = a.counts[level];
  uint32_t*      loc   = FIRST ? a.loc1 : a.loc2;
  uint32_t*      tile  = FIRST ? a.tile1 : a.tile2;
  if ( !FIRST ) {
    for ( uint32_t s = blockIdx.x * blockDim.x + threadIdx.x; s < count; s += gridDim.x * blockDim.x ) {
      const LvSeg* q = cur + s;
      if ( !( q->cutInfo >> 24 ) ) continue;
      for ( int c = 0; c < 2; ++c )
        for ( int d = 0; d < 3; ++d ) next[q->slot + c].mn[d] = 0x7FFFFFFF, next[q->slot + c].mx[d] = int32_t( 0x80000000 );
    }
  }
  for ( uint32_t t = blockIdx.x; t < tiles; t += gridDim.x ) {
    const uint32_t base = t * kScanTile + threadIdx.x * 8;
    uint32_t       v[8], run = 0;
#pragma unroll
    for ( int k = 0; k < 8; ++k ) {
      const uint32_t i = base + k;
      uint32_t       f = 0;
      if ( i < n ) {
        const uint32_t s = a.seg[i];
        if ( s != kNone ) {
          const LvSeg*   q  = cur + s;
          const uint32_t ci = q->cutInfo;
          if ( ci >> 24 ) {
            const int32_t c = int32_t( int16_t( ci & 0xFFFFu ) ), x = coordOf( a.P[i], int( ( ci >> 16 ) & 0xFFu ) );
            f               = FIRST ? uint32_t( x >= c ) : uint32_t( i >= q->edge1 && x > c );
          }
        }
      }
      v[k] = f;
      run += f;
    }
    uint32_t inc = run;
#pragma unroll
    for ( int off = 1; off < 64; off <<= 1 ) {
      const uint32_t u = __shfl_up( inc, off, 64 );
      if ( lane >= off ) inc += u;
    }
    if ( lane == 63 ) waveSum[wave] = inc;
    __syncthreads();
    uint32_t offset = inc - run;
    for ( int w = 0; w < wave; ++w ) offset += waveSum[w];
#pragma unroll
    for ( int k = 0; k < 8; ++k ) {
      if ( base + k < n ) {
        loc[base + k] = offset;
        if ( !v[k] ) a.list[size_t( t ) * kScanTile + ( threadIdx.x * 8 + k - offset )] = uint16_t( threadIdx.x * 8 + k );
      }
      offset += v[k];
    }
    if ( threadIdx.x == kBlock - 1 ) tile[t] = offset;
    __syncthreads();
  }
}

template <int BLOCK>
__device__ __forceinline__ void lvLoadSums( uint32_t* sums, const uint32_t* __restrict__ raw, uint32_t tiles ) {
  __shared__ uint32_t waveSum[BLOCK / 64];
  const int lane = threadIdx.x & 63, wave = threadIdx.x >> 6;
  uint32_t  carry = 0;
  for ( uint32_t base = 0; base < tiles; base += BLOCK ) {
    const uint32_t i   = base + threadIdx.x;
    const uint32_t v   = i < tiles ? raw[i] : 0u;
    uint32_t       inc = v;
#pragma unroll
    for ( int off = 1; off < 64; off <<= 1 ) {
      const uint32_t u = __shfl_up( inc, off, 64 );
      if ( lane >= off ) inc += u;
    }
    if ( lane == 63 ) waveSum[wave] = inc;
    __syncthreads();
    uint32_t offset = carry + inc - v;
    for ( int w = 0; w < wave; ++w ) offset += waveSum[w];
    if ( i < tiles ) sums[i] = offset;
    for ( int w = 0; w < BLOCK / 64; ++w ) carry += waveSum[w];
    __syncthreads();
  }
  if ( threadIdx.x == 0 ) sums[tiles] = carry;
  __syncthreads();
}

__global__ __launch_bounds__( kBlock ) void lvSwapOneKernel( BuildArgs a, uint32_t level ) {
  extern __shared__ uint32_t lvSums[];
  const uint32_t n = a.n, tiles = a.tiles;
  const uint32_t gsize = gridDim.x * blockDim.x;
  LvSeg*         cur = ( level & 1 ) ? a.lvB : a.lvA;
  lvLoadSums<kBlock>( lvSums, a.tile1, tiles );
  for ( uint32_t i = blockIdx.x * blockDim.x + threadIdx.x; i < n; i += gsize ) {
    const uint32_t s = a.seg[i];
    if ( s == kNone ) continue;
    LvSeg*         q  = cur + s;
    const uint32_t ci = q->cutInfo;
    if ( !( ci >> 24 ) ) continue;
    const uint32_t b = q->begin, e = q->end;
    const Pt       pi = a.P[i];
    const uint32_t li = a.loc1[i];
    const uint32_t rb = lvPrefix( a.loc1, lvSums, tiles, b, n ), re = lvPrefix( a.loc1, lvSums, tiles, e, n );
    const uint32_t edge = b + ( ( e - b ) - ( re - rb ) );
    if ( i == b ) q->edge1 = edge;
    if ( i >= edge || coordOf( pi, int( ( ci >> 16 ) & 0xFFu ) ) < int32_t( int16_t( ci & 0xFFFFu ) ) ) continue;
    const uint32_t r  = li + lvSums[i / kScanTile] - rb;
    const uint32_t j  = lvPartner( a.list, lvSums, edge, e, ( e - re ) - 1u - r );
    const Pt       pj = a.P[j];
    a.P[i]            = pj;
    a.P[j]            = pi;
    const uint32_t u  = a.perm[i];
    a.perm[i]         = a.perm[j];
    a.perm[j]         = u;
  }
}

__global__ __launch_bounds__( kLandBlock ) void lvSwapTwoKernel( BuildArgs a, uint32_t level ) {
  extern __shared__ uint32_t lvSums[];
  const uint32_t n = a.n, tiles = a.tiles;
  const int      lane  = threadIdx.x & 63;
  LvSeg*         cur  = ( level & 1 ) ? a.lvB : a.lvA;
  LvSeg*         next = ( level & 1 ) ? a.lvA : a.lvB;
  lvLoadSums<kLandBlock>( lvSums, a.tile2, tiles );
  const uint32_t nRound = ( n + uint32_t( kLandBlock ) - 1u ) & ~( uint32_t( kLandBlock ) - 1u );
  __shared__ uint32_t blockSeg;
  __shared__ uint32_t red[kLandBlock / 64][6];
  __shared__ uint32_t accV[6], accSlot;
  const int wave = threadIdx.x >> 6;
  constexpr uint32_t kChunk = uint32_t( kLandBlock ) * kLandRounds;
  for ( uint32_t c0 = blockIdx.x * kChunk; c0 < nRound; c0 += gridDim.x * kChunk ) {
  if ( threadIdx.x == 0 ) accSlot = kNone;
  for ( uint32_t i0 = c0; i0 < min( c0 + kChunk, nRound ); i0 += kLandBlock ) {
    const uint32_t i   = i0 + threadIdx.x;
    uint32_t       key = kNoKey;
    uint32_t       A = pk2( 0x7FFF, 0x7FFF ), B = pk2( -0x8000, -0x8000 ), C = pk2( 0x7FFF, 0x7FFF );
    uint32_t       A2 = A, B2 = B, C2 = C;
    bool           moved = false;
    uint32_t       s = kNone, slot = 0;
    if ( i < n ) {
      s           = a.seg[i];
      uint32_t to = kNone;
      if ( s != kNone ) {
        LvSeg*         q  = cur + s;
        const uint32_t ci = q->cutInfo;
        if ( ci >> 24 ) {
          const uint32_t b = q->begin, e = q->end, e1 = q->edge1;
          slot               = q->slot;
          const int      dim = int( ( ci >> 16 ) & 0xFFu );
          const int32_t  cut = int32_t( int16_t( ci & 0xFFFFu ) );
          Pt             pi  = a.P[i];
          const uint32_t li  = a.loc2[i];
          const uint32_t rb = lvPrefix( a.loc2, lvSums, tiles, e1, n ), re = lvPrefix( a.loc2, lvSums, tiles, e, n );
          const uint32_t e2   = e1 + ( ( e - e1 ) - ( re - rb ) );
          const uint32_t cnt  = e - b, half = cnt / 2, lim1 = e1 - b, lim2 = e2 - b;
          const uint32_t idx  = lim1 > half ? lim1 : ( lim2 < half ? lim2 : half );
          const uint32_t mid  = b + idx;
          if ( i == b ) {
            KdNode nd;
            nd.a = int32_t( q->childNode ), nd.b = int32_t( q->childNode + 1u ), nd.divlow = nd.divhigh = 0, nd.dim = dim;
            a.nodes[q->node] = nd;
            for ( int c = 0; c < 2; ++c ) {
              LvSeg* ch = next + slot + c;
              ch->begin = c ? mid : b, ch->end = c ? e : mid, ch->cutInfo = 0, ch->edge1 = 0, ch->slot = 0, ch->childNode = 0;
              ch->node = q->childNode + c, ch->parent = q->node, ch->side = uint8_t( c ), ch->pdim = uint8_t( dim ), ch->unused = 0;
              for ( int d = 0; d < 3; ++d ) ch->lo[d] = q->lo[d], ch->hi[d] = q->hi[d];
              if ( c == 0 ) {
                if ( dim == 0 ) ch->hi[0] = int16_t( cut );
                if ( dim == 1 ) ch->hi[1] = int16_t( cut );
                if ( dim == 2 ) ch->hi[2] = int16_t( cut );
              } else {
                if ( dim == 0 ) ch->lo[0] = int16_t( cut );
                if ( dim == 1 ) ch->lo[1] = int16_t( cut );
                if ( dim == 2 ) ch->lo[2] = int16_t( cut );
              }
            }
          }
          const int32_t x = coordOf( pi, dim );
          to              = slot + ( i >= mid ? 1u : 0u );
          key             = to;
          if ( i >= e1 && i < e2 && x > cut ) {
            const uint32_t r  = li + lvSums[i / kScanTile] - rb;
            const uint32_t j  = lvPartner( a.list, lvSums, e2, e, ( e - re ) - 1u - r );
            const Pt       pj = a.P[j];
            a.P[i]            = pj;
            a.P[j]            = pi;
            const uint32_t u  = a.perm[i];
            a.perm[i]         = a.perm[j];
            a.perm[j]         = u;
            moved             = true;
            A2 = pk2( pi.x, pi.y ), B2 = A2, C2 = pk2( pi.z, ~int( pi.z ) );
            pi = pj;
          }
          if ( !( i >= e2 && x <= cut ) ) A = pk2( pi.x, pi.y ), B = A, C = pk2( pi.z, ~int( pi.z ) );
        }
        a.seg[i] = to;
      }
    }
    if ( threadIdx.x == 0 ) blockSeg = s;
    __syncthreads();
    const bool uniform = __syncthreads_and( s == blockSeg ) != 0;
    if ( uniform ) {
      const bool anything = __syncthreads_or( key != kNoKey ) != 0;
      if ( anything ) {
        uint32_t v[6];
        const bool right = key != kNoKey && key != slot;
        v[0] = right || key == kNoKey ? pk2( 0x7FFF, 0x7FFF ) : A, v[1] = right || key == kNoKey ? pk2( -0x8000, -0x8000 ) : B,
        v[2] = right || key == kNoKey ? pk2( 0x7FFF, 0x7FFF ) : C;
        v[3] = pkMin( right ? A : pk2( 0x7FFF, 0x7FFF ), A2 ), v[4] = pkMax( right ? B : pk2( -0x8000, -0x8000 ), B2 ),
        v[5] = pkMin( right ? C : pk2( 0x7FFF, 0x7FFF ), C2 );
#pragma unroll
        for ( int off = 32; off > 0; off >>= 1 ) {
          v[0] = pkMin( v[0], __shfl_xor( v[0], off, 64 ) ), v[1] = pkMax( v[1], __shfl_xor( v[1], off, 64 ) ), v[2] = pkMin( v[2], __shfl_xor( v[2], off, 64 ) );
          v[3] = pkMin( v[3], __shfl_xor( v[3], off, 64 ) ), v[4] = pkMax( v[4], __shfl_xor( v[4], off, 64 ) ), v[5] = pkMin( v[5], __shfl_xor( v[5], off, 64 ) );
        }
        if ( lane == 0 )
          for ( int k = 0; k < 6; ++k ) red[wave][k] = v[k];
        __syncthreads();
        if ( threadIdx.x == 0 ) {
          uint32_t x[6];
          for ( int k = 0; k < 6; ++k ) {
            x[k] = red[0][k];
            for ( int w = 1; w < kLandBlock / 64; ++w ) x[k] = ( k % 3 ) == 1 ? pkMax( x[k], red[w][k] ) : pkMin( x[k], red[w][k] );
          }
          if ( accSlot != kNone && accSlot != slot ) {
            for ( int c = 0; c < 2; ++c )
              lvReport( next + accSlot + c, pkLo( accV[3 * c] ), pkHi( accV[3 * c] ), pkLo( accV[3 * c + 2] ), pkLo( accV[3 * c + 1] ), pkHi( accV[3 * c + 1] ),
                        ~pkHi( accV[3 * c + 2] ) );
            accSlot = kNone;
          }
          for ( int k = 0; k < 6; ++k ) accV[k] = accSlot == kNone ? x[k] : ( ( k % 3 ) == 1 ? pkMax( accV[k], x[k] ) : pkMin( accV[k], x[k] ) );
          accSlot = slot;
        }
      }
      __syncthreads();
      continue;
    }
    if ( moved ) lvReport( next + slot + 1u, pkLo( A2 ), pkHi( A2 ), pkLo( C2 ), pkLo( A2 ), pkHi( A2 ), pkLo( C2 ) );
    if ( waveSegMinMaxPacked( key, A, B, C, lane ) )
      lvReport( next + key, pkLo( A ), pkHi( A ), pkLo( C ), pkLo( B ), pkHi( B ), ~pkHi( C ) );
  }
  __syncthreads();
  if ( threadIdx.x == 0 ) {
    LvPartial pt;
    pt.slot = accSlot, pt.unused = 0;
    for ( int k = 0; k < 6; ++k ) pt.v[k] = accV[k];
    a.partial[c0 / kChunk] = pt;
  }
  __syncthreads();
  }
}

constexpr size_t kPieceLdsBytes = size_t( kPieceMax ) * ( sizeof( Pt ) + 4 + 2 + 2 + 2 ) + 16 + 2 * size_t( kPieceRecs ) * sizeof( PieceRec );

constexpr int kPiecePer = 4;
template <bool PROFILE = false>
__global__ __launch_bounds__( kPieceMax / kPiecePer ) void pieceKernel( BuildArgs a ) {
  unsigned long long profLast = 0, prof[12] = {0, 0, 0, 0, 0, 0, 0, 0, 0, 0, 0, 0};
#define PIECE_MARK( k )                                        \
  if ( PROFILE && threadIdx.x == 0 ) {                         \
    const unsigned long long now_ = wall_clock64();            \
    prof[k] += now_ - profLast, profLast = now_;               \
  }
  constexpr int K = kPiecePer, THREADS = kPieceMax / K, WAVES = THREADS / 64;
  extern __shared__ __align__( 16 ) unsigned char pieceLds[];
  Pt*       P     = reinterpret_cast<Pt*>( pieceLds );
  uint32_t* perm  = reinterpret_cast<uint32_t*>( P + kPieceMax );
  uint16_t* pre   = reinterpret_cast<uint16_t*>( perm + kPieceMax );
  uint16_t* lst   = pre + kPieceMax + 8;
  uint16_t* segOf = lst + kPieceMax;
  PieceRec* recs  = reinterpret_cast<PieceRec*>( segOf + kPieceMax );
  __shared__ __align__( 16 ) uint32_t sWave[2][WAVES];
  __shared__ uint32_t sCount[2], sNodeBase, sDepth;
  const int      lane = threadIdx.x & 63, tid = threadIdx.x;
  const uint32_t total = *a.retiredCount;
  const uint32_t p0    = uint32_t( tid ) * K;
  for ( uint32_t s = blockIdx.x; s < total; s += gridDim.x ) {
    const RetiredSeg seg = a.retired[s];
    const uint32_t   cnt = seg.end - seg.begin;
    uint32_t idPending   = 0;
    if ( tid == 0 ) idPending = atomicAdd( a.nodeCount, 2u );
    pieceBarrier();
    for ( uint32_t i = tid; i < uint32_t( kPieceMax ); i += THREADS ) {
      if ( i < cnt ) {
        P[i]     = a.P[seg.begin + i];
        perm[i]  = a.perm[seg.begin + i];
        segOf[i] = 0;
      } else {
        segOf[i] = kNoRec;
      }
    }
    if ( tid == 0 ) {
      PieceRec r{};
      r.begin = 0, r.end = uint16_t( cnt ), r.node = seg.node;
      for ( int d = 0; d < 3; ++d ) r.lo[d] = seg.lo[d], r.hi[d] = seg.hi[d], r.mn[d] = 0x7FFFFFFF, r.mx[d] = int32_t( 0x80000000 );
      recs[0]   = r;
      sCount[0] = 1, sCount[1] = 0, sDepth = 0;
    }
    pieceBarrier();
    {
      uint32_t A = pk2( 0x7FFF, 0x7FFF ), B = pk2( -0x8000, -0x8000 ), C = pk2( 0x7FFF, 0x7FFF );
      bool     any = false;
#pragma unroll
      for ( int k = 0; k < K; ++k ) {
        const uint32_t p = p0 + k;
        if ( p < cnt ) {
          const Pt x = P[p];
          A = pkMin( A, pk2( x.x, x.y ) ), B = pkMax( B, pk2( x.x, x.y ) ), C = pkMin( C, pk2( x.z, ~int( x.z ) ) );
          any = true;
        }
      }
      if ( waveSegMinMaxPacked( any ? 0u : kNoKey, A, B, C, lane ) ) {
        ldsMin( &recs[0].mn[0], pkLo( A ) ), ldsMin( &recs[0].mn[1], pkHi( A ) ), ldsMin( &recs[0].mn[2], pkLo( C ) );
        ldsMax( &recs[0].mx[0], pkLo( B ) ), ldsMax( &recs[0].mx[1], pkHi( B ) ), ldsMax( &recs[0].mx[2], ~pkHi( C ) );
      }
    }
    pieceBarrier();
    if ( seg.root != 0 && tid == 0 ) {
      for ( int d = 0; d < 3; ++d ) {
        recs[0].lo[d] = int16_t( recs[0].mn[d] ), recs[0].hi[d] = int16_t( recs[0].mx[d] );
        a.rootBox[d] = recs[0].mn[d], a.rootBox[3 + d] = recs[0].mx[d];
      }
    }
    if ( PROFILE && threadIdx.x == 0 ) profLast = wall_clock64();
    uint32_t deepest  = 0;
    uint32_t prevBase = 0, prevCount = 0;
    int      cur      = 0;
    for ( uint32_t depth = 0;; ++depth ) {
      pieceBarrier();
      PIECE_MARK( 0 )
      const uint32_t nc = sCount[cur];
      PieceRec*      R  = recs + cur * kPieceRecs;
      PieceRec*      RN = recs + ( cur ^ 1 ) * kPieceRecs;
      for ( uint32_t r = tid; r < prevCount; r += THREADS ) {
        const PieceRec* q = RN + r;
        KdNode          nd;
        nd.a = int32_t( prevBase + 2u * r ), nd.b = int32_t( prevBase + 2u * r + 1u ), nd.divlow = int16_t( q->lmax ), nd.divhigh = int16_t( q->rmin ),
        nd.dim = q->dim;
        a.nodes[q->node] = nd;
      }
      if ( nc == 0 ) break;
      if ( seg.level + depth >= uint32_t( kMaxLevels ) - 2u ) {
        if ( tid == 0 ) atomicMax( a.finishDepth, 0x10000u );
        break;
      }
      if ( tid == 0 ) sNodeBase = idPending, sCount[cur ^ 1] = 0;
      for ( uint32_t r = tid; r < nc; r += THREADS ) {
        PieceRec*     q   = R + r;
        const int32_t lo0 = q->lo[0], lo1 = q->lo[1], lo2 = q->lo[2], hi0 = q->hi[0], hi1 = q->hi[1], hi2 = q->hi[2];
        const int32_t mn0 = q->mn[0], mn1 = q->mn[1], mn2 = q->mn[2], mx0 = q->mx[0], mx1 = q->mx[1], mx2 = q->mx[2];
        const int32_t maxSpan = max( hi0 - lo0, max( hi1 - lo1, hi2 - lo2 ) );
        const double  limit   = ( 1.0 - 0.00001 ) * double( maxSpan );
        int           dim     = 0;
        int32_t       best    = -1;
        if ( double( hi0 - lo0 ) > limit && mx0 - mn0 > best ) best = mx0 - mn0, dim = 0;
        if ( double( hi1 - lo1 ) > limit && mx1 - mn1 > best ) best = mx1 - mn1, dim = 1;
        if ( double( hi2 - lo2 ) > limit && mx2 - mn2 > best ) best = mx2 - mn2, dim = 2;
        const int32_t l = dim == 0 ? lo0 : ( dim == 1 ? lo1 : lo2 ), h = dim == 0 ? hi0 : ( dim == 1 ? hi1 : hi2 );
        const int32_t lowest = dim == 0 ? mn0 : ( dim == 1 ? mn1 : mn2 ), highest = dim == 0 ? mx0 : ( dim == 1 ? mx1 : mx2 );
        q->dim = uint8_t( dim ), q->unused0 = 0, q->cut = int16_t( min( max( ( l + h ) / 2, lowest ), highest ) );
      }
      pieceBarrier();
      PIECE_MARK( 1 )
      uint32_t rec[K], be[K], dc[K];
      bool     waveLive = true;
      {
        uint16_t raw[K];
        *reinterpret_cast<uint2*>( raw ) = *reinterpret_cast<const uint2*>( segOf + p0 );
        bool same = true, live = false;
#pragma unroll
        for ( int k = 0; k < K; ++k ) rec[k] = raw[k], same = same && raw[k] == raw[0], live = live || raw[k] != kNoRec;
        waveLive = __ballot( live ) != 0ull;
        if ( same ) {
          PieceHot0 h{0, 0};
          if ( rec[0] != kNoRec ) h = *reinterpret_cast<const PieceHot0*>( R + rec[0] );
#pragma unroll
          for ( int k = 0; k < K; ++k ) be[k] = h.be, dc[k] = h.dc;
        } else {
#pragma unroll
          for ( int k = 0; k < K; ++k ) {
            PieceHot0 h{0, 0};
            if ( rec[k] != kNoRec ) h = *reinterpret_cast<const PieceHot0*>( R + rec[k] );
            be[k] = h.be, dc[k] = h.dc;
          }
        }
      }
      uint32_t f1 = 0;
      if ( waveLive ) {
        Pt x[K];
#pragma unroll
        for ( int k = 0; k < K; k += 2 ) *reinterpret_cast<uint4*>( &x[k] ) = *reinterpret_cast<const uint4*>( P + p0 + k );
#pragma unroll
        for ( int k = 0; k < K; ++k ) {
          const int d = int( ( dc[k] >> 16 ) & 0xFFu ), c = int( int16_t( dc[k] & 0xFFFFu ) );
          const int v = int( int16_t( __builtin_bit_cast( uint64_t, x[k] ) >> ( 16 * d ) ) );
          if ( rec[k] != kNoRec && v >= c ) f1 |= 1u << k;
        }
      }
      uint32_t preA[K + 1];
      {
        uint32_t at = pieceScan<WAVES>( uint32_t( __popc( f1 ) ), sWave[0] );
        uint16_t out[K];
#pragma unroll
        for ( int k = 0; k < K; ++k ) preA[k] = at, out[k] = uint16_t( at ), at += ( f1 >> k ) & 1u;
        preA[K] = at;
        *reinterpret_cast<uint2*>( pre + p0 ) = *reinterpret_cast<const uint2*>( out );
        if ( tid == THREADS - 1 ) pre[kPieceMax] = uint16_t( at );
      }
      pieceBarrier();
      PIECE_MARK( 2)
      uint32_t edge1[K], rb1[K];
#pragma unroll
      for ( int k = 0; k < K; ++k ) {
        edge1[k] = rb1[k] = 0;
        if ( !waveLive || rec[k] == kNoRec ) continue;
        if ( k > 0 && rec[k] == rec[k - 1] ) {
          edge1[k] = edge1[k - 1], rb1[k] = rb1[k - 1];
        } else {
          const uint32_t b = be[k] & 0xFFFFu, e = be[k] >> 16, rb = pre[b], re = pre[e];
          edge1[k] = b + ( ( e - b ) - ( re - rb ) ), rb1[k] = rb | ( re << 16 );
        }
        const uint32_t p = p0 + k, b = be[k] & 0xFFFFu, e = be[k] >> 16;
        if ( p >= edge1[k] && !( ( f1 >> k ) & 1u ) ) lst[b + ( ( e - p - 1u ) - ( ( rb1[k] >> 16 ) - preA[k + 1] ) )] = uint16_t( p );
        if ( p == b ) *reinterpret_cast<uint32_t*>( &R[rec[k]].edge1 ) = edge1[k] | ( ( rb1[k] & 0xFFFFu ) << 16 );
      }
      pieceBarrier();
      PIECE_MARK( 3)
#pragma unroll
      for ( int k = 0; k < K; ++k ) {
        const uint32_t p = p0 + k;
        if ( waveLive && rec[k] != kNoRec && p < edge1[k] && ( ( f1 >> k ) & 1u ) ) {
          const uint32_t j  = lst[( be[k] & 0xFFFFu ) + ( preA[k] - ( rb1[k] & 0xFFFFu ) )];
          const Pt       px = P[p], pj = P[j];
          const uint32_t ip = perm[p], ij = perm[j];
          P[p] = pj, P[j] = px, perm[p] = ij, perm[j] = ip;
        }
      }
      pieceBarrier();
      PIECE_MARK( 4)
      uint32_t f2 = 0;
      if ( waveLive ) {
        Pt x[K];
#pragma unroll
        for ( int k = 0; k < K; k += 2 ) *reinterpret_cast<uint4*>( &x[k] ) = *reinterpret_cast<const uint4*>( P + p0 + k );
#pragma unroll
        for ( int k = 0; k < K; ++k ) {
          const int d = int( ( dc[k] >> 16 ) & 0xFFu ), c = int( int16_t( dc[k] & 0xFFFFu ) );
          const int v = int( int16_t( __builtin_bit_cast( uint64_t, x[k] ) >> ( 16 * d ) ) );
          if ( rec[k] != kNoRec && p0 + k >= edge1[k] && v > c ) f2 |= 1u << k;
        }
      }
      {
        uint32_t at = pieceScan<WAVES>( uint32_t( __popc( f2 ) ), sWave[1] );
        uint16_t out[K];
#pragma unroll
        for ( int k = 0; k < K; ++k ) preA[k] = at, out[k] = uint16_t( at ), at += ( f2 >> k ) & 1u;
        preA[K] = at;
        *reinterpret_cast<uint2*>( pre + p0 ) = *reinterpret_cast<const uint2*>( out );
        if ( tid == THREADS - 1 ) pre[kPieceMax] = uint16_t( at );
      }
      pieceBarrier();
      PIECE_MARK( 5)
      const uint32_t base = sNodeBase;
      for ( uint32_t r = tid; r < nc; r += THREADS ) {
        PieceRec*      q  = R + r;
        const uint32_t b = q->begin, e = q->end, e1 = q->edge1, rb2 = pre[e1], re2 = pre[e];
        const uint32_t e2   = e1 + ( ( e - e1 ) - ( re2 - rb2 ) );
        const uint32_t n    = e - b, half = n / 2, lim1 = e1 - b, lim2 = e2 - b;
        const uint32_t idx  = lim1 > half ? lim1 : ( lim2 < half ? lim2 : half );
        const uint32_t mid  = b + idx;
        const uint32_t id0  = base + 2u * r;
        const int      dim  = q->dim;
        const int16_t  cut  = q->cut;
        q->edge2 = uint16_t( e2 ), q->rb2 = uint16_t( rb2 ), q->mid = uint16_t( mid );
        q->lmax = int32_t( 0x80000000 ), q->rmin = 0x7FFFFFFF;
#pragma unroll
        for ( int c = 0; c < 2; ++c ) {
          const uint32_t cb = c ? mid : b, ce = c ? e : mid;
          if ( ce - cb <= uint32_t( kLeafMax ) ) {
            KdNode leaf;
            leaf.a = int32_t( seg.begin + cb ), leaf.b = int32_t( seg.begin + ce ), leaf.divlow = leaf.divhigh = 0, leaf.dim = -1;
            a.nodes[id0 + c] = leaf;
            q->child[c]      = kNoRec;
            deepest          = max( deepest, seg.level + depth + 2u );
          } else {
            const uint32_t slot = atomicAdd( &sCount[cur ^ 1], 1u );
            PieceRec*      ch   = RN + slot;
            ch->begin = uint16_t( cb ), ch->end = uint16_t( ce ), ch->node = id0 + c;
            int16_t l0 = q->lo[0], l1 = q->lo[1], l2 = q->lo[2], h0 = q->hi[0], h1 = q->hi[1], h2 = q->hi[2];
            if ( c == 0 ) {
              if ( dim == 0 ) h0 = cut;
              if ( dim == 1 ) h1 = cut;
              if ( dim == 2 ) h2 = cut;
            } else {
              if ( dim == 0 ) l0 = cut;
              if ( dim == 1 ) l1 = cut;
              if ( dim == 2 ) l2 = cut;
            }
            ch->lo[0] = l0, ch->lo[1] = l1, ch->lo[2] = l2, ch->hi[0] = h0, ch->hi[1] = h1, ch->hi[2] = h2;
            ch->mn[0] = ch->mn[1] = ch->mn[2] = 0x7FFFFFFF, ch->mx[0] = ch->mx[1] = ch->mx[2] = int32_t( 0x80000000 );
            q->child[c] = uint16_t( slot );
          }
        }
      }
      uint32_t edge2[K], rb2[K];
#pragma unroll
      for ( int k = 0; k < K; ++k ) {
        edge2[k] = rb2[k] = 0;
        if ( !waveLive || rec[k] == kNoRec ) continue;
        const uint32_t e = be[k] >> 16, e1 = edge1[k];
        if ( k > 0 && rec[k] == rec[k - 1] ) {
          edge2[k] = edge2[k - 1], rb2[k] = rb2[k - 1];
        } else {
          const uint32_t rb = pre[e1], re = pre[e];
          edge2[k] = e1 + ( ( e - e1 ) - ( re - rb ) ), rb2[k] = rb | ( re << 16 );
        }
        const uint32_t p = p0 + k;
        if ( p >= edge2[k] && !( ( f2 >> k ) & 1u ) ) lst[e1 + ( ( e - p - 1u ) - ( ( rb2[k] >> 16 ) - preA[k + 1] ) )] = uint16_t( p );
      }
      pieceBarrier();
      PIECE_MARK( 6)
      prevBase = base, prevCount = nc;
      if ( tid == 0 && sCount[cur ^ 1] ) idPending = atomicAdd( a.nodeCount, 2u * sCount[cur ^ 1] );
#pragma unroll
      for ( int k = 0; k < K; ++k ) {
        const uint32_t p = p0 + k;
        if ( waveLive && rec[k] != kNoRec && p >= edge1[k] && p < edge2[k] && ( ( f2 >> k ) & 1u ) ) {
          const uint32_t j  = lst[edge1[k] + ( preA[k] - ( rb2[k] & 0xFFFFu ) )];
          const Pt       px = P[p], pj = P[j];
          const uint32_t ip = perm[p], ij = perm[j];
          P[p] = pj, P[j] = px, perm[p] = ij, perm[j] = ip;
        }
      }
      pieceBarrier();
      PIECE_MARK( 7)
      if ( waveLive ) {
        uint32_t key[K], mc[K], c1[K];
        bool     same = true;
#pragma unroll
        for ( int k = 0; k < K; ++k ) {
          mc[k] = c1[k] = 0;
          if ( rec[k] != kNoRec ) {
            if ( k > 0 && rec[k] == rec[k - 1] ) {
              mc[k] = mc[k - 1], c1[k] = c1[k - 1];
            } else {
              const PieceHot2 h = *reinterpret_cast<const PieceHot2*>( &R[rec[k]].mid );
              mc[k] = h.midc0, c1[k] = h.c1 & 0xFFFFu;
            }
          }
          key[k] = rec[k] == kNoRec ? kNoKey : 2u * rec[k] + ( p0 + k >= ( mc[k] & 0xFFFFu ) ? 1u : 0u );
          same   = same && key[k] == key[0];
        }
        Pt x[K];
#pragma unroll
        for ( int k = 0; k < K; k += 2 ) *reinterpret_cast<uint4*>( &x[k] ) = *reinterpret_cast<const uint4*>( P + p0 + k );
        uint32_t A = pk2( 0x7FFF, 0x7FFF ), B = pk2( -0x8000, -0x8000 ), C = pk2( 0x7FFF, 0x7FFF );
        if ( same && key[0] != kNoKey ) {
#pragma unroll
          for ( int k = 0; k < K; ++k )
            A = pkMin( A, pk2( x[k].x, x[k].y ) ), B = pkMax( B, pk2( x[k].x, x[k].y ) ), C = pkMin( C, pk2( x[k].z, ~int( x[k].z ) ) );
        }
        const bool head = waveSegMinMaxPacked( same ? key[0] : kNoKey, A, B, C, lane );
        uint16_t out[K];
#pragma unroll
        for ( int k = 0; k < K; ++k ) {
          out[k] = kNoRec;
          if ( key[k] == kNoKey ) continue;
          const uint32_t side = key[k] & 1u;
          const uint32_t cr   = side ? c1[k] : ( mc[k] >> 16 );
          out[k]              = uint16_t( cr );
          if ( same ? ( k > 0 || !head ) : false ) continue;
          int mnx, mny, mnz, mxx, mxy, mxz;
          if ( same )
            mnx = pkLo( A ), mny = pkHi( A ), mnz = pkLo( C ), mxx = pkLo( B ), mxy = pkHi( B ), mxz = ~pkHi( C );
          else
            mnx = mxx = x[k].x, mny = mxy = x[k].y, mnz = mxz = x[k].z;
          PieceRec* q = R + rec[k];
          const int d = int( ( dc[k] >> 16 ) & 0xFFu );
          if ( side == 0 )
            ldsMax( &q->lmax, d == 0 ? mxx : ( d == 1 ? mxy : mxz ) );
          else
            ldsMin( &q->rmin, d == 0 ? mnx : ( d == 1 ? mny : mnz ) );
          if ( cr != kNoRec ) {
            PieceRec* ch = RN + cr;
            ldsMin( &ch->mn[0], mnx ), ldsMin( &ch->mn[1], mny ), ldsMin( &ch->mn[2], mnz );
            ldsMax( &ch->mx[0], mxx ), ldsMax( &ch->mx[1], mxy ), ldsMax( &ch->mx[2], mxz );
          }
        }
        *reinterpret_cast<uint2*>( segOf + p0 ) = *reinterpret_cast<const uint2*>( out );
      }
      cur ^= 1;
    }
    if ( deepest ) atomicMax( &sDepth, deepest );
    if ( PROFILE && threadIdx.x == 0 ) {
      for ( int k = 0; k < 8; ++k ) atomicAdd( a.pieceProfile + k, prof[k] ), prof[k] = 0;
      atomicAdd( a.pieceProfile + 8, 1ull );
    }
    pieceBarrier();
    for ( uint32_t i = tid; i < cnt; i += THREADS ) {
      a.P[seg.begin + i]    = P[i];
      a.perm[seg.begin + i] = perm[i];
    }
    if ( tid == 0 && sDepth ) atomicMax( a.finishDepth, sDepth );
  }
  if ( a.hostDepth && tid == 0 ) {
    __threadfence();
    if ( atomicAdd( a.ticket, 1u ) == gridDim.x - 1u ) {
      __threadfence();
      *a.hostDepth = __hip_atomic_load( a.finishDepth, __ATOMIC_RELAXED, __HIP_MEMORY_SCOPE_AGENT );
    }
  }
}

}

int buildKdTreeDevice( tmc2_ctx* ctx, const Pt* d_pts, uint64_t n64, DeviceTree& tree ) {
  const uint32_t n = uint32_t( n64 );
  tree.n           = n64;
  tree.depth       = 0;
  for ( int d = 0; d < 3; ++d ) tree.lo[d] = tree.hi[d] = 0;
  if ( n == 0 ) return TMC2_OK;
  hipStream_t    s       = ctx->stream;
  const uint32_t tiles   = ( n + kScanTile - 1 ) / kScanTile;
  const size_t   maxSegs = 2 * ( size_t( n ) / ( kLeafMax + 1 ) + 1 ) + 2;
  const size_t   maxNode = 2 * size_t( n ) + 2;
  TMC2_TRY( tree.ptsTree.alloc( n ) );
  TMC2_TRY( tree.perm.alloc( n ) );
  TMC2_TRY( tree.nodes.alloc( maxNode ) );
  DevBuf<uint32_t>   d_work, d_small;
  DevBuf<BuildSeg>   d_segs;
  DevBuf<RetiredSeg> d_retired;
  const size_t       maxRetired = size_t( n ) / ( kLeafMax + 1 ) + 2;
  TMC2_TRY( d_retired.alloc( maxRetired ) );
  DevBuf<HugeSeg> d_huge;
  TMC2_TRY( d_huge.alloc( size_t( n ) / ( kPieceMax + 1 ) + 2 ) );
  const auto     hugeEnv = ctxOption( ctx, "KD_HUGEMAX" );
  const uint32_t hugeMax = std::min<uint32_t>( kHugeLimit, std::max<uint32_t>( kPieceMax, hugeEnv ? uint32_t( atoi( hugeEnv->c_str() ) ) : 16384u ) );
  TMC2_TRY( d_work.alloc( 3 * size_t( n ) + 2 * ( size_t( tiles ) + 1 ) ) );
  TMC2_TRY( d_segs.alloc( 2 * maxSegs ) );
  TMC2_TRY( d_small.alloc( kMaxLevels + 16 ) );
  static_assert( kMaxLevels + 16 <= 128, "lvRootKernel clears the counters with one workgroup of 128" );
  BuildArgs a;
  a.pts = d_pts, a.n = n, a.tiles = tiles, a.P = tree.ptsTree.p, a.perm = tree.perm.p;
  a.seg = d_work.p, a.loc1 = d_work.p + n, a.loc2 = d_work.p + 2 * size_t( n );
  a.tile1 = d_work.p + 3 * size_t( n ), a.tile2 = a.tile1 + tiles + 1;
  a.segA = d_segs.p, a.segB = d_segs.p + maxSegs, a.nodes = tree.nodes.p;
  a.counts    = d_small.p;
  a.nodeCount = d_small.p + kMaxLevels + 1;
  a.levels    = d_small.p + kMaxLevels + 2;
  a.rootBox   = reinterpret_cast<int32_t*>( d_small.p + kMaxLevels + 8 );
  a.retired      = d_retired.p;
  a.retiredCount = d_small.p + kMaxLevels + 3;
  a.finishDepth  = d_small.p + kMaxLevels + 4;
  a.ticket       = d_small.p + kMaxLevels + 5;
  a.bigCount     = d_small.p + kMaxLevels + 6;
  a.huge         = d_huge.p;
  a.hugeCount    = d_small.p + kMaxLevels + 7;
  a.hugeMax      = hugeMax;
  a.hostSmall    = nullptr;
  a.hostDepth    = ctx->answerLine( tmc2_ctx::kAnswerTreeDepth );
  a.retireMax    = uint32_t( kPieceMax );
  a.splitMax     = uint32_t( kPieceMax );
  const dim3 blk( kBlock ), grdE( std::max<uint32_t>( 1u, ( n + 2 * kBlock - 1 ) / ( 2 * kBlock ) ) ), grdT( tiles );
  const dim3 grdL( std::max<uint32_t>( 1u, ( n + kLandBlock * kLandRounds - 1 ) / ( kLandBlock * kLandRounds ) ) );
  const size_t sumsLds = ( size_t( tiles ) + 1 ) * 4;
  if ( sumsLds > 48 * 1024 ) {
    setError( "kdtree: %u points -- the level passes hold one word per 2 048-point tile in LDS (at most 25 M points)", n );
    return TMC2_E_UNSUPPORTED;
  }
  DevBuf<LvSeg>    d_lv;
  DevBuf<uint16_t> d_list;
  DevBuf<LvPartial> d_partial;
  const size_t     maxLv = 2 * ( size_t( n ) / ( size_t( kPieceMax ) + 1 ) + 2 );
  TMC2_TRY( d_lv.alloc( 2 * maxLv ) );
  TMC2_TRY( d_list.alloc( size_t( tiles ) * kScanTile ) );
  TMC2_TRY( d_partial.alloc( size_t( n ) / ( kLandBlock * kLandRounds ) + 2 ) );
  a.lvA = d_lv.p, a.lvB = d_lv.p + maxLv, a.list = d_list.p, a.partial = d_partial.p;
  const auto decideOpt = ctxOption( ctx, "KD_DECIDE" );
  a.decideRng = decideOpt && ( *decideOpt )[0] == 'g' ? 0u : uint32_t( kDecideRng );
  hipLaunchKernelGGL( lvRootKernel, dim3( 1 ), dim3( 128 ), 0, s, a );
  hipLaunchKernelGGL( lvInitKernel, dim3( std::min<uint32_t>( grdE.x, 1024u ) ), blk, 0, s, a );
  hipLaunchKernelGGL( lvDecideKernel, dim3( 1 ), dim3( kDecideThreads ), 0, s, a, 0u );
  uint32_t out[kMaxLevels + 16];
  int      found = -1;
  int& hint = ctx->kdLevelHint[( n >> 15 ) * 2u + 1u];
  for ( uint32_t level = 0; level < uint32_t( kMaxLevels ) && found < 0; ) {
    uint32_t chunkEnd = level + 1;
    if ( level == 0 && hint > 0 ) {
      chunkEnd = uint32_t( std::min( hint, kMaxLevels ) );
    } else {
      while ( chunkEnd < uint32_t( kMaxLevels ) && ( uint64_t( hugeMax ) << std::min<uint32_t>( chunkEnd - 1, 40 ) ) < n ) ++chunkEnd;
      if ( chunkEnd == level + 1 ) chunkEnd = std::min<uint32_t>( level + 2, kMaxLevels );
    }
    volatile uint32_t* hostSmall = ctx->answerLine( tmc2_ctx::kAnswerTreeLevels );
    for ( ; level < chunkEnd; ++level ) {
      hipLaunchKernelGGL( lvFlagKernel<true>, grdT, blk, 0, s, a, level );
      hipLaunchKernelGGL( lvSwapOneKernel, grdE, blk, sumsLds, s, a, level );
      hipLaunchKernelGGL( lvFlagKernel<false>, grdT, blk, 0, s, a, level );
      hipLaunchKernelGGL( lvSwapTwoKernel, grdL, dim3( kLandBlock ), sumsLds, s, a, level );
      BuildArgs ad = a;
      if ( level + 1 == chunkEnd ) ad.hostSmall = hostSmall;
      hipLaunchKernelGGL( lvDecideKernel, dim3( 1 ), dim3( kDecideThreads ), 0, s, ad, level + 1u );
    }
    TMC2_HIP( hipGetLastError() );
    TMC2_HIP( hipStreamSynchronize( s ) );
    for ( int w = 0; w < kMaxLevels + 16; ++w ) out[w] = hostSmall[w];
    for ( uint32_t l = 0; l <= level && l <= uint32_t( kMaxLevels ); ++l )
      if ( out[l] == 0 ) {
        found = int( l );
        break;
      }
  }
  if ( found < 0 ) {
    setError( "kdtree: more than %d levels", kMaxLevels - 1 );
    return TMC2_E_UNSUPPORTED;
  }
  tree.depth = found;
  hint       = std::max( found, 1 );
  const int32_t* box = reinterpret_cast<const int32_t*>( out + kMaxLevels + 8 );
  for ( int d = 0; d < 3; ++d ) tree.lo[d] = box[d], tree.hi[d] = box[3 + d];
  const uint32_t hugeSegs = out[kMaxLevels + 7];
  if ( hugeSegs )
    hipLaunchKernelGGL( hugeSegmentsKernel, dim3( std::min<uint32_t>( hugeSegs, 4u * uint32_t( ctx->cuCount ) ) ), dim3( 64 * kHugeWaves ), 0, s, a );
  const uint32_t retired = out[kMaxLevels + 3] + hugeSegs * ( 2u * hugeMax / uint32_t( kPieceMax ) );
  if ( retired ) {
    const dim3 grid( std::min<uint32_t>( retired, 8u * uint32_t( ctx->cuCount ) ) ), block( kPieceMax / kPiecePer );
    if ( ctxOption( ctx, "KD_PIECE_PROFILE" ) ) {
      DevBuf<unsigned long long> d_prof;
      TMC2_TRY( d_prof.alloc( 16 ) );
      TMC2_HIP( hipMemsetAsync( d_prof.p, 0, 16 * 8, s ) );
      a.pieceProfile = d_prof.p;
      TMC2_TRY( allowLargeLds( reinterpret_cast<const void*>( pieceKernel<true> ), kPieceLdsBytes, ctx->device, 256 ) );
      hipLaunchKernelGGL( pieceKernel<true>, grid, block, kPieceLdsBytes, s, a );
      unsigned long long h[16];
      TMC2_HIP( hipMemcpyAsync( h, d_prof.p, sizeof( h ), hipMemcpyDeviceToHost, s ) );
      TMC2_HIP( hipStreamSynchronize( s ) );
      static const char* what[8] = {"landing of the previous depth", "node records + split rules", "first flags + prefix sum", "first publish",
                                    "first swaps", "second flags + prefix sum", "children + second publish", "second swaps"};
      fprintf( stderr, "pieceKernel: %llu pieces, us per piece between the barriers of its depths (thread 0 of each workgroup):", h[8] );
      for ( int k = 0; k < 8; ++k ) fprintf( stderr, " %s %.1f |", what[k], 0.01 * double( h[k] ) / double( std::max<unsigned long long>( h[8], 1 ) ) );
      fprintf( stderr, "\n" );
    } else {
      TMC2_TRY( allowLargeLds( reinterpret_cast<const void*>( pieceKernel<> ), kPieceLdsBytes, ctx->device, 256 ) );
      hipLaunchKernelGGL( pieceKernel<>, grid, block, kPieceLdsBytes, s, a );
    }
    TMC2_HIP( hipGetLastError() );
    TMC2_HIP( hipStreamSynchronize( s ) );
    const uint32_t fin = *a.hostDepth;
    if ( fin >= uint32_t( kMaxLevels ) ) {
      setError( "kdtree: more than %d levels", kMaxLevels - 1 );
      return TMC2_E_UNSUPPORTED;
    }
    tree.depth = std::max( tree.depth, int( fin ) );
  }
  return TMC2_OK;
}

}
```

Measured before the change: 193.3.

## Restructure GPU kd-tree build: fused start, pull-based partition, speculative piece launch

```diff
diff --git a/mpeg-pcc-tmc2_amd/csrc/api.cpp b/mpeg-pcc-tmc2_amd/csrc/api.cpp
--- a/mpeg-pcc-tmc2_amd/csrc/api.cpp
+++ b/mpeg-pcc-tmc2_amd/csrc/api.cpp
@@ -293,7 +293,7 @@
     return TMC2_E_INVALID;
   }
   tmc2::ApiScope scope( ctx );
-  const uint64_t perPoint = voxelDimRefine > 0 && voxelDimRefine <= 2 ? 5500 : 2400;
+  const uint64_t perPoint = voxelDimRefine > 0 && voxelDimRefine <= 2 ? 5532 : 2432;
   const int      gridShift = std::max( 1, bits3d - 1 - ( voxelDimRefine >= 4 ? 2 : ( voxelDimRefine >= 2 ? 1 : 0 ) ) );
   const uint64_t dense     = ( uint64_t( 1 ) << std::min( 33, 3 * gridShift + 1 ) ) / 32 * 8;
   const uint64_t bytes     = maxPoints * perPoint + uint64_t( maxCanvasWidth ) * uint64_t( maxCanvasHeight ) * 64 + dense + ( uint64_t( 64 ) << 20 );
@@ -365,6 +365,7 @@
     ApiScope scope( ctx );
     ctx->gridBits.release();
     ctx->scanState.release();
+    ctx->kdTicket.release();
     ctx->voxelBitmap.release();
     ctx->constTables.clear();
     ctx->retiredTables.clear();
diff --git a/mpeg-pcc-tmc2_amd/csrc/internal.h b/mpeg-pcc-tmc2_amd/csrc/internal.h
--- a/mpeg-pcc-tmc2_amd/csrc/internal.h
+++ b/mpeg-pcc-tmc2_amd/csrc/internal.h
@@ -262,6 +262,12 @@
   uint32_t                      scanEpoch = 0, scanTickets = 0;
   tmc2::DevBuf<uint32_t>        voxelBitmap;
   std::map<uint32_t, int>       kdLevelHint;
+  struct KdGridHint {
+    uint32_t v[2] = {0, 0};
+  };
+  std::map<uint32_t, KdGridHint> kdGridHint;
+  tmc2::DevBuf<uint32_t>        kdTicket;
+  uint32_t                      kdTickets = 0;
   struct ConstTable {
     tmc2::DevBuf<int> dev;
     std::vector<int>  host;
diff --git a/mpeg-pcc-tmc2_amd/csrc/kdtree_device.hip b/mpeg-pcc-tmc2_amd/csrc/kdtree_device.hip
--- a/mpeg-pcc-tmc2_amd/csrc/kdtree_device.hip
+++ b/mpeg-pcc-tmc2_amd/csrc/kdtree_device.hip
@@ -43,6 +43,8 @@
   uint32_t  n, tiles;
   Pt*       P;
   uint32_t *perm, *seg;
+  Pt*       P2;
+  uint32_t* perm2;
   BuildSeg *segA, *segB;
   KdNode*   nodes;
   uint32_t *loc1, *loc2, *tile1, *tile2;
@@ -58,7 +60,10 @@
   uint32_t    hugeMax;
   uint32_t    retireMax, splitMax;
   struct LvSeg *lvA, *lvB;
-  uint16_t*   list;
+  uint16_t *  list, *list2;
+  int32_t*    startRng;
+  uint32_t*   startTicket;
+  uint32_t    specLevel;
   struct LvPartial* partial;
   unsigned long long* pieceProfile;
   uint32_t    decideRng;
@@ -176,6 +181,7 @@
   __shared__ uint32_t sCount[2], waveCnt[2 * kHugeWaves];
   __shared__ int32_t  red[kHugeWaves][12];
   const int      lane = threadIdx.x & 63, wave = threadIdx.x >> 6;
+  if ( a.specLevel != kNone && a.counts[a.specLevel] != 0 ) return;
   const uint32_t total = *a.hugeCount;
   for ( uint32_t s = blockIdx.x; s < total; s += gridDim.x ) {
     const HugeSeg seg = a.huge[s];
@@ -422,8 +428,82 @@
   return lo * kScanTile + list[size_t( lo ) * kScanTile + ( G - ( lo * kScanTile - sums[lo] ) )];
 }
 
-__global__ __launch_bounds__( kBlock ) void lvInitKernel( BuildArgs a ) {
-  __shared__ int blockRange[6 * kWaves];
+__device__ __forceinline__ uint32_t lvClassAt( const uint16_t* __restrict__ list, const uint32_t* sums, uint32_t from, uint32_t to, uint32_t G ) {
+  uint32_t lo = from / kScanTile, hi = ( to - 1u ) / kScanTile;
+  while ( lo < hi ) {
+    const uint32_t mid = ( lo + hi + 1u ) / 2u;
+    if ( sums[mid] <= G )
+      lo = mid;
+    else
+      hi = mid - 1u;
+  }
+  return lo * kScanTile + list[size_t( lo ) * kScanTile + ( uint32_t( kScanTile ) - 1u - ( ( G - sums[lo] ) & ( uint32_t( kScanTile ) - 1u ) ) )];
+}
+
+template <bool ALONE>
+__device__ __forceinline__ uint32_t lvDecideSegment( const BuildArgs& a, LvSeg* q, uint32_t level, const int32_t ( &mn )[3], const int32_t ( &mx )[3] ) {
+  const bool root = q->parent == kNone;
+  int32_t    lo[3], hi[3];
+#pragma unroll
+  for ( int d = 0; d < 3; ++d ) {
+    lo[d] = root ? mn[d] : int32_t( q->lo[d] );
+    hi[d] = root ? mx[d] : int32_t( q->hi[d] );
+  }
+  if ( root ) {
+    for ( int d = 0; d < 3; ++d ) a.rootBox[d] = mn[d], a.rootBox[3 + d] = mx[d];
+  } else {
+    const int pd = q->pdim;
+    if ( q->side == 0 )
+      a.nodes[q->parent].divlow = int16_t( pd == 0 ? mx[0] : ( pd == 1 ? mx[1] : mx[2] ) );
+    else
+      a.nodes[q->parent].divhigh = int16_t( pd == 0 ? mn[0] : ( pd == 1 ? mn[1] : mn[2] ) );
+  }
+  const uint32_t cnt = q->end - q->begin;
+  if ( cnt <= uint32_t( kLeafMax ) ) {
+    KdNode nd;
+    nd.a = int32_t( q->begin ), nd.b = int32_t( q->end ), nd.divlow = nd.divhigh = 0, nd.dim = -1;
+    a.nodes[q->node] = nd;
+  } else if ( cnt <= a.retireMax ) {
+    RetiredSeg r;
+    r.begin = q->begin, r.end = q->end, r.node = q->node, r.level = level;
+    r.root  = root ? 1 : 0;
+    for ( int d = 0; d < 3; ++d ) r.lo[d] = q->lo[d], r.hi[d] = q->hi[d];
+    if ( ALONE )
+      a.retired[0] = r, *a.retiredCount = 1;
+    else
+      a.retired[atomicAdd( a.retiredCount, 1u )] = r;
+  } else if ( cnt <= a.hugeMax ) {
+    HugeSeg r;
+    r.begin = q->begin, r.end = q->end, r.node = q->node, r.level = level;
+    r.root  = root ? 1 : 0;
+    for ( int d = 0; d < 3; ++d ) r.lo[d] = q->lo[d], r.hi[d] = q->hi[d], r.mn[d] = mn[d], r.mx[d] = mx[d];
+    if ( ALONE )
+      a.huge[0] = r, *a.hugeCount = 1;
+    else
+      a.huge[atomicAdd( a.hugeCount, 1u )] = r;
+  } else {
+    const int32_t maxSpan = max( hi[0] - lo[0], max( hi[1] - lo[1], hi[2] - lo[2] ) );
+    const double  limit   = ( 1.0 - 0.00001 ) * double( maxSpan );
+    int           dim     = 0;
+    int32_t       best    = -1;
+    if ( double( hi[0] - lo[0] ) > limit && mx[0] - mn[0] > best ) best = mx[0] - mn[0], dim = 0;
+    if ( double( hi[1] - lo[1] ) > limit && mx[1] - mn[1] > best ) best = mx[1] - mn[1], dim = 1;
+    if ( double( hi[2] - lo[2] ) > limit && mx[2] - mn[2] > best ) best = mx[2] - mn[2], dim = 2;
+    const int32_t l = dim == 0 ? lo[0] : ( dim == 1 ? lo[1] : lo[2] ), h = dim == 0 ? hi[0] : ( dim == 1 ? hi[1] : hi[2] );
+    const int32_t lowest = dim == 0 ? mn[0] : ( dim == 1 ? mn[1] : mn[2] ), highest = dim == 0 ? mx[0] : ( dim == 1 ? mx[1] : mx[2] );
+    const int32_t cut = min( max( ( l + h ) / 2, lowest ), highest );
+    q->cutInfo = ( uint32_t( cut ) & 0xFFFFu ) | ( uint32_t( dim ) << 16 ) | ( 1u << 24 );
+    if ( root )
+      for ( int d = 0; d < 3; ++d ) q->lo[d] = int16_t( mn[d] ), q->hi[d] = int16_t( mx[d] );
+    return 1;
+  }
+  q->cutInfo = 0;
+  return 0;
+}
+
+__global__ __launch_bounds__( kBlock ) void lvStartKernel( BuildArgs a, uint32_t ticketBase ) {
+  __shared__ int  blockRange[6 * kWaves];
+  __shared__ bool isLast;
   const uint32_t n = a.n, gsize = gridDim.x * blockDim.x;
   const int      lane = threadIdx.x & 63, wave = threadIdx.x >> 6;
   int mnx = 0x7FFFFFFF, mny = mnx, mnz = mnx, mxx = int( 0x80000000 ), mxy = mxx, mxz = mxx;
@@ -448,24 +528,50 @@
   if ( threadIdx.x < 6 ) {
     int v = blockRange[threadIdx.x];
     for ( int w = 1; w < kWaves; ++w ) v = threadIdx.x < 3 ? min( v, blockRange[6 * w + threadIdx.x] ) : max( v, blockRange[6 * w + threadIdx.x] );
-    int32_t* slot = threadIdx.x < 3 ? &a.lvA[0].mn[threadIdx.x] : &a.lvA[0].mx[threadIdx.x - 3];
-    if ( threadIdx.x < 3 ) {
-      if ( v < loadStaleOk( slot ) ) atomicMin( slot, v );
-    } else {
-      if ( v > loadStaleOk( slot ) ) atomicMax( slot, v );
-    }
-  }
-}
-__global__ void lvRootKernel( BuildArgs a ) {
+    __hip_atomic_store( &a.startRng[6u * blockIdx.x + threadIdx.x], v, __ATOMIC_RELAXED, __HIP_MEMORY_SCOPE_AGENT );
+    asm volatile( "s_waitcnt vmcnt(0)" ::: "memory" );
+  }
+  __syncthreads();
+  if ( threadIdx.x == 0 ) isLast = __hip_atomic_fetch_add( a.startTicket, 1u, __ATOMIC_RELAXED, __HIP_MEMORY_SCOPE_AGENT ) - ticketBase == gridDim.x - 1u;
+  __syncthreads();
+  if ( !isLast ) return;
+  static_assert( kMaxLevels + 16 <= kBlock, "the last workgroup clears the counters with one store per thread" );
   if ( threadIdx.x < kMaxLevels + 16 ) a.counts[threadIdx.x] = 0;
+  int r[6];
+#pragma unroll
+  for ( int k = 0; k < 6; ++k ) r[k] = k < 3 ? 0x7FFFFFFF : int( 0x80000000 );
+  for ( uint32_t b = threadIdx.x; b < gridDim.x; b += blockDim.x )
+#pragma unroll
+    for ( int k = 0; k < 6; ++k ) {
+      const int v = __hip_atomic_load( &a.startRng[6u * b + k], __ATOMIC_RELAXED, __HIP_MEMORY_SCOPE_AGENT );
+      r[k]        = k < 3 ? min( r[k], v ) : max( r[k], v );
+    }
+#pragma unroll
+  for ( int off = 32; off > 0; off >>= 1 )
+#pragma unroll
+    for ( int k = 0; k < 6; ++k ) {
+      const int o = __shfl_xor( r[k], off, 64 );
+      r[k]        = k < 3 ? min( r[k], o ) : max( r[k], o );
+    }
+  if ( lane == 0 )
+    for ( int k = 0; k < 6; ++k ) blockRange[6 * wave + k] = r[k];
   __syncthreads();
   if ( threadIdx.x != 0 ) return;
-  LvSeg r{};
-  r.begin = 0, r.end = a.n, r.node = 0, r.parent = kNone;
-  for ( int d = 0; d < 3; ++d ) r.mn[d] = 0x7FFFFFFF, r.mx[d] = int32_t( 0x80000000 );
-  a.lvA[0]     = r;
-  a.counts[0]  = 1;
-  *a.nodeCount = 1;
+  LvSeg root{};
+  root.begin = 0, root.end = n, root.node = 0, root.parent = kNone;
+  for ( int k = 0; k < 6; ++k ) {
+    int v = blockRange[k];
+    for ( int w = 1; w < kWaves; ++w ) v = k < 3 ? min( v, blockRange[6 * w + k] ) : max( v, blockRange[6 * w + k] );
+    ( k < 3 ? root.mn[k] : root.mx[k - 3] ) = v;
+  }
+  a.lvA[0]                = root;
+  const int32_t  mn[3]    = {root.mn[0], root.mn[1], root.mn[2]}, mx[3] = {root.mx[0], root.mx[1], root.mx[2]};
+  const uint32_t split    = lvDecideSegment<true>( a, &a.lvA[0], 0u, mn, mx );
+  a.lvA[0].slot           = 0;
+  a.lvA[0].childNode      = 1;
+  a.counts[0]             = 1;
+  a.counts[1]             = 2u * split;
+  *a.nodeCount            = 1u + 2u * split;
 }
 
 constexpr int kDecideThreads = 1024;
@@ -512,59 +618,14 @@
     uint32_t       split = 0;
     LvSeg*         q     = cur + s;
     if ( s < count ) {
-      const bool root = q->parent == kNone;
-      int32_t    mn[3], mx[3], lo[3], hi[3];
+      int32_t mn[3], mx[3];
 #pragma unroll
       for ( int d = 0; d < 3; ++d ) {
         mn[d] = __hip_atomic_load( &q->mn[d], __ATOMIC_RELAXED, __HIP_MEMORY_SCOPE_AGENT );
         mx[d] = __hip_atomic_load( &q->mx[d], __ATOMIC_RELAXED, __HIP_MEMORY_SCOPE_AGENT );
         if ( inLds ) mn[d] = min( mn[d], sRng[s][d] ), mx[d] = max( mx[d], sRng[s][3 + d] );
-        lo[d] = root ? mn[d] : int32_t( q->lo[d] );
-        hi[d] = root ? mx[d] : int32_t( q->hi[d] );
-      }
-      if ( root ) {
-        for ( int d = 0; d < 3; ++d ) a.rootBox[d] = mn[d], a.rootBox[3 + d] = mx[d];
-      } else {
-        const int pd = q->pdim;
-        if ( q->side == 0 )
-          a.nodes[q->parent].divlow = int16_t( pd == 0 ? mx[0] : ( pd == 1 ? mx[1] : mx[2] ) );
-        else
-          a.nodes[q->parent].divhigh = int16_t( pd == 0 ? mn[0] : ( pd == 1 ? mn[1] : mn[2] ) );
-      }
-      const uint32_t cnt = q->end - q->begin;
-      if ( cnt <= uint32_t( kLeafMax ) ) {
-        KdNode nd;
-        nd.a = int32_t( q->begin ), nd.b = int32_t( q->end ), nd.divlow = nd.divhigh = 0, nd.dim = -1;
-        a.nodes[q->node] = nd;
-      } else if ( cnt <= a.retireMax ) {
-        RetiredSeg r;
-        r.begin = q->begin, r.end = q->end, r.node = q->node, r.level = level;
-        r.root  = root ? 1 : 0;
-        for ( int d = 0; d < 3; ++d ) r.lo[d] = q->lo[d], r.hi[d] = q->hi[d];
-        a.retired[atomicAdd( a.retiredCount, 1u )] = r;
-      } else if ( cnt <= a.hugeMax ) {
-        HugeSeg r;
-        r.begin = q->begin, r.end = q->end, r.node = q->node, r.level = level;
-        r.root  = root ? 1 : 0;
-        for ( int d = 0; d < 3; ++d ) r.lo[d] = q->lo[d], r.hi[d] = q->hi[d], r.mn[d] = mn[d], r.mx[d] = mx[d];
-        a.huge[atomicAdd( a.hugeCount, 1u )] = r;
-      } else {
-        const int32_t maxSpan = max( hi[0] - lo[0], max( hi[1] - lo[1], hi[2] - lo[2] ) );
-        const double  limit   = ( 1.0 - 0.00001 ) * double( maxSpan );
-        int           dim     = 0;
-        int32_t       best    = -1;
-        if ( double( hi[0] - lo[0] ) > limit && mx[0] - mn[0] > best ) best = mx[0] - mn[0], dim = 0;
-        if ( double( hi[1] - lo[1] ) > limit && mx[1] - mn[1] > best ) best = mx[1] - mn[1], dim = 1;
-        if ( double( hi[2] - lo[2] ) > limit && mx[2] - mn[2] > best ) best = mx[2] - mn[2], dim = 2;
-        const int32_t l = dim == 0 ? lo[0] : ( dim == 1 ? lo[1] : lo[2] ), h = dim == 0 ? hi[0] : ( dim == 1 ? hi[1] : hi[2] );
-        const int32_t lowest = dim == 0 ? mn[0] : ( dim == 1 ? mn[1] : mn[2] ), highest = dim == 0 ? mx[0] : ( dim == 1 ? mx[1] : mx[2] );
-        const int32_t cut = min( max( ( l + h ) / 2, lowest ), highest );
-        q->cutInfo = ( uint32_t( cut ) & 0xFFFFu ) | ( uint32_t( dim ) << 16 ) | ( 1u << 24 );
-        if ( root )
-          for ( int d = 0; d < 3; ++d ) q->lo[d] = int16_t( mn[d] ), q->hi[d] = int16_t( mx[d] );
-        split = 1;
-      }
-      if ( !split ) q->cutInfo = 0;
+      }
+      split = lvDecideSegment<false>( a, q, level, mn, mx );
     }
     uint32_t inc = split;
 #pragma unroll
@@ -596,24 +657,11 @@
   }
 }
 
-template <bool FIRST>
 __global__ __launch_bounds__( kBlock ) void lvFlagKernel( BuildArgs a, uint32_t level ) {
   __shared__ uint32_t waveSum[kWaves];
   const uint32_t n = a.n, tiles = a.tiles;
   const int      lane = threadIdx.x & 63, wave = threadIdx.x >> 6;
   LvSeg*         cur   = ( level & 1 ) ? a.lvB : a.lvA;
-  LvSeg*         next  = ( level & 1 ) ? a.lvA : a.lvB;
-  const uint32_t count = a.counts[level];
-  uint32_t*      loc   = FIRST ? a.loc1 : a.loc2;
-  uint32_t*      tile  = FIRST ? a.tile1 : a.tile2;
-  if ( !FIRST ) {
-    for ( uint32_t s = blockIdx.x * blockDim.x + threadIdx.x; s < count; s += gridDim.x * blockDim.x ) {
-      const LvSeg* q = cur + s;
-      if ( !( q->cutInfo >> 24 ) ) continue;
-      for ( int c = 0; c < 2; ++c )
-        for ( int d = 0; d < 3; ++d ) next[q->slot + c].mn[d] = 0x7FFFFFFF, next[q->slot + c].mx[d] = int32_t( 0x80000000 );
-    }
-  }
   for ( uint32_t t = blockIdx.x; t < tiles; t += gridDim.x ) {
     const uint32_t base = t * kScanTile + threadIdx.x * 8;
     uint32_t       v[8], run = 0;
@@ -624,12 +672,8 @@
       if ( i < n ) {
         const uint32_t s = a.seg[i];
         if ( s != kNone ) {
-          const LvSeg*   q  = cur + s;
-          const uint32_t ci = q->cutInfo;
-          if ( ci >> 24 ) {
-            const int32_t c = int32_t( int16_t( ci & 0xFFFFu ) ), x = coordOf( a.P[i], int( ( ci >> 16 ) & 0xFFu ) );
-            f               = FIRST ? uint32_t( x >= c ) : uint32_t( i >= q->edge1 && x > c );
-          }
+          const uint32_t ci = cur[s].cutInfo;
+          if ( ci >> 24 ) f = uint32_t( coordOf( a.P[i], int( ( ci >> 16 ) & 0xFFu ) ) >= int32_t( int16_t( ci & 0xFFFFu ) ) );
         }
       }
       v[k] = f;
@@ -645,15 +689,16 @@
     __syncthreads();
     uint32_t offset = inc - run;
     for ( int w = 0; w < wave; ++w ) offset += waveSum[w];
+    uint16_t* tl = a.list + size_t( t ) * kScanTile;
 #pragma unroll
     for ( int k = 0; k < 8; ++k ) {
       if ( base + k < n ) {
-        loc[base + k] = offset;
-        if ( !v[k] ) a.list[size_t( t ) * kScanTile + ( threadIdx.x * 8 + k - offset )] = uint16_t( threadIdx.x * 8 + k );
+        a.loc1[base + k] = offset;
+        tl[v[k] ? uint32_t( kScanTile ) - 1u - offset : threadIdx.x * 8 + k - offset] = uint16_t( threadIdx.x * 8 + k );
       }
       offset += v[k];
     }
-    if ( threadIdx.x == kBlock - 1 ) tile[t] = offset;
+    if ( threadIdx.x == kBlock - 1 ) a.tile1[t] = offset;
     __syncthreads();
   }
 }
@@ -684,37 +729,95 @@
   __syncthreads();
 }
 
-__global__ __launch_bounds__( kBlock ) void lvSwapOneKernel( BuildArgs a, uint32_t level ) {
+__global__ __launch_bounds__( kBlock ) void lvPullOneKernel( BuildArgs a, uint32_t level ) {
   extern __shared__ uint32_t lvSums[];
+  __shared__ uint32_t waveSum[kWaves];
   const uint32_t n = a.n, tiles = a.tiles;
-  const uint32_t gsize = gridDim.x * blockDim.x;
-  LvSeg*         cur = ( level & 1 ) ? a.lvB : a.lvA;
+  const int      lane = threadIdx.x & 63, wave = threadIdx.x >> 6;
+  LvSeg*         cur   = ( level & 1 ) ? a.lvB : a.lvA;
+  LvSeg*         next  = ( level & 1 ) ? a.lvA : a.lvB;
+  const uint32_t count = a.counts[level];
   lvLoadSums<kBlock>( lvSums, a.tile1, tiles );
-  for ( uint32_t i = blockIdx.x * blockDim.x + threadIdx.x; i < n; i += gsize ) {
-    const uint32_t s = a.seg[i];
-    if ( s == kNone ) continue;
-    LvSeg*         q  = cur + s;
-    const uint32_t ci = q->cutInfo;
-    if ( !( ci >> 24 ) ) continue;
-    const uint32_t b = q->begin, e = q->end;
-    const Pt       pi = a.P[i];
-    const uint32_t li = a.loc1[i];
-    const uint32_t rb = lvPrefix( a.loc1, lvSums, tiles, b, n ), re = lvPrefix( a.loc1, lvSums, tiles, e, n );
-    const uint32_t edge = b + ( ( e - b ) - ( re - rb ) );
-    if ( i == b ) q->edge1 = edge;
-    if ( i >= edge || coordOf( pi, int( ( ci >> 16 ) & 0xFFu ) ) < int32_t( int16_t( ci & 0xFFFFu ) ) ) continue;
-    const uint32_t r  = li + lvSums[i / kScanTile] - rb;
-    const uint32_t j  = lvPartner( a.list, lvSums, edge, e, ( e - re ) - 1u - r );
-    const Pt       pj = a.P[j];
-    a.P[i]            = pj;
-    a.P[j]            = pi;
-    const uint32_t u  = a.perm[i];
-    a.perm[i]         = a.perm[j];
-    a.perm[j]         = u;
-  }
-}
-
-__global__ __launch_bounds__( kLandBlock ) void lvSwapTwoKernel( BuildArgs a, uint32_t level ) {
+  for ( uint32_t s = blockIdx.x * blockDim.x + threadIdx.x; s < count; s += gridDim.x * blockDim.x ) {
+    const LvSeg* q = cur + s;
+    if ( !( q->cutInfo >> 24 ) ) continue;
+    for ( int c = 0; c < 2; ++c )
+      for ( int d = 0; d < 3; ++d ) next[q->slot + c].mn[d] = 0x7FFFFFFF, next[q->slot + c].mx[d] = int32_t( 0x80000000 );
+  }
+  for ( uint32_t t = blockIdx.x; t < tiles; t += gridDim.x ) {
+    const uint32_t base = t * kScanTile + threadIdx.x * 8;
+    uint32_t from[8], rule[8];
+    LvSeg*   first     = nullptr;
+    uint32_t firstEdge = 0;
+#pragma unroll
+    for ( int k = 0; k < 8; ++k ) {
+      const uint32_t i = base + k;
+      from[k] = i, rule[k] = 0;
+      if ( i < n ) {
+        const uint32_t s = a.seg[i];
+        if ( s != kNone ) {
+          LvSeg*         q  = cur + s;
+          const uint32_t ci = q->cutInfo;
+          if ( ci >> 24 ) {
+            const uint32_t b = q->begin, e = q->end;
+            const uint32_t li = a.loc1[i] + lvSums[t];
+            const uint32_t rb = lvPrefix( a.loc1, lvSums, tiles, b, n ), re = lvPrefix( a.loc1, lvSums, tiles, e, n );
+            const uint32_t edge = b + ( ( e - b ) - ( re - rb ) );
+            if ( i == b ) first = q, firstEdge = edge;
+            const bool ge = coordOf( a.P[i], int( ( ci >> 16 ) & 0xFFu ) ) >= int32_t( int16_t( ci & 0xFFFFu ) );
+            if ( i < edge && ge )
+              from[k] = lvPartner( a.list, lvSums, edge, e, ( e - re ) - 1u - ( li - rb ) );
+            else if ( i >= edge && !ge )
+              from[k] = lvClassAt( a.list, lvSums, b, edge, rb + ( ( e - i - 1u ) - ( re - li ) ) );
+            from[k] = min( from[k], n - 1u );
+            rule[k] = ( ci & 0xFFFFFFu ) | ( i >= edge ? 1u << 24 : 0u ) | ( 1u << 25 );
+          }
+        }
+      }
+    }
+    Pt       land[8];
+    uint32_t id[8];
+#pragma unroll
+    for ( int k = 0; k < 8; ++k )
+      if ( rule[k] ) land[k] = a.P[from[k]], id[k] = a.perm[from[k]];
+    if ( first ) first->edge1 = firstEdge;
+    uint32_t v[8], run = 0;
+#pragma unroll
+    for ( int k = 0; k < 8; ++k ) {
+      uint32_t f = 0;
+      if ( rule[k] ) {
+        a.P2[base + k]    = land[k];
+        a.perm2[base + k] = id[k];
+        f = uint32_t( ( rule[k] >> 24 & 1u ) && coordOf( land[k], int( ( rule[k] >> 16 ) & 0xFFu ) ) > int32_t( int16_t( rule[k] & 0xFFFFu ) ) );
+      }
+      v[k] = f;
+      run += f;
+    }
+    uint32_t inc = run;
+#pragma unroll
+    for ( int off = 1; off < 64; off <<= 1 ) {
+      const uint32_t u = __shfl_up( inc, off, 64 );
+      if ( lane >= off ) inc += u;
+    }
+    if ( lane == 63 ) waveSum[wave] = inc;
+    __syncthreads();
+    uint32_t offset = inc - run;
+    for ( int w = 0; w < wave; ++w ) offset += waveSum[w];
+    uint16_t* tl = a.list2 + size_t( t ) * kScanTile;
+#pragma unroll
+    for ( int k = 0; k < 8; ++k ) {
+      if ( base + k < n ) {
+        a.loc2[base + k] = offset;
+        tl[v[k] ? uint32_t( kScanTile ) - 1u - offset : threadIdx.x * 8 + k - offset] = uint16_t( threadIdx.x * 8 + k );
+      }
+      offset += v[k];
+    }
+    if ( threadIdx.x == kBlock - 1 ) a.tile2[t] = offset;
+    __syncthreads();
+  }
+}
+
+__global__ __launch_bounds__( kLandBlock ) void lvPullTwoKernel( BuildArgs a, uint32_t level ) {
   extern __shared__ uint32_t lvSums[];
   const uint32_t n = a.n, tiles = a.tiles;
   const int      lane  = threadIdx.x & 63;
@@ -733,8 +836,6 @@
     const uint32_t i   = i0 + threadIdx.x;
     uint32_t       key = kNoKey;
     uint32_t       A = pk2( 0x7FFF, 0x7FFF ), B = pk2( -0x8000, -0x8000 ), C = pk2( 0x7FFF, 0x7FFF );
-    uint32_t       A2 = A, B2 = B, C2 = C;
-    bool           moved = false;
     uint32_t       s = kNone, slot = 0;
     if ( i < n ) {
       s           = a.seg[i];
@@ -747,8 +848,8 @@
           slot               = q->slot;
           const int      dim = int( ( ci >> 16 ) & 0xFFu );
           const int32_t  cut = int32_t( int16_t( ci & 0xFFFFu ) );
-          Pt             pi  = a.P[i];
-          const uint32_t li  = a.loc2[i];
+          Pt             pi  = a.P2[i];
+          const uint32_t li  = a.loc2[i] + lvSums[i / kScanTile];
           const uint32_t rb = lvPrefix( a.loc2, lvSums, tiles, e1, n ), re = lvPrefix( a.loc2, lvSums, tiles, e, n );
           const uint32_t e2   = e1 + ( ( e - e1 ) - ( re - rb ) );
           const uint32_t cnt  = e - b, half = cnt / 2, lim1 = e1 - b, lim2 = e2 - b;
@@ -777,20 +878,16 @@
           const int32_t x = coordOf( pi, dim );
           to              = slot + ( i >= mid ? 1u : 0u );
           key             = to;
-          if ( i >= e1 && i < e2 && x > cut ) {
-            const uint32_t r  = li + lvSums[i / kScanTile] - rb;
-            const uint32_t j  = lvPartner( a.list, lvSums, e2, e, ( e - re ) - 1u - r );
-            const Pt       pj = a.P[j];
-            a.P[i]            = pj;
-            a.P[j]            = pi;
-            const uint32_t u  = a.perm[i];
-            a.perm[i]         = a.perm[j];
-            a.perm[j]         = u;
-            moved             = true;
-            A2 = pk2( pi.x, pi.y ), B2 = A2, C2 = pk2( pi.z, ~int( pi.z ) );
-            pi = pj;
-          }
-          if ( !( i >= e2 && x <= cut ) ) A = pk2( pi.x, pi.y ), B = A, C = pk2( pi.z, ~int( pi.z ) );
+          uint32_t from   = i;
+          if ( i >= e1 && i < e2 && x > cut )
+            from = lvPartner( a.list2, lvSums, e2, e, ( e - re ) - 1u - ( li - rb ) );
+          else if ( i >= e2 && x <= cut )
+            from = lvClassAt( a.list2, lvSums, e1, e2, rb + ( ( e - i - 1u ) - ( re - li ) ) );
+          from = min( from, n - 1u );
+          if ( from != i ) pi = a.P2[from];
+          a.P[i]    = pi;
+          a.perm[i] = a.perm2[from];
+          A = pk2( pi.x, pi.y ), B = A, C = pk2( pi.z, ~int( pi.z ) );
         }
         a.seg[i] = to;
       }
@@ -805,8 +902,7 @@
         const bool right = key != kNoKey && key != slot;
         v[0] = right || key == kNoKey ? pk2( 0x7FFF, 0x7FFF ) : A, v[1] = right || key == kNoKey ? pk2( -0x8000, -0x8000 ) : B,
         v[2] = right || key == kNoKey ? pk2( 0x7FFF, 0x7FFF ) : C;
-        v[3] = pkMin( right ? A : pk2( 0x7FFF, 0x7FFF ), A2 ), v[4] = pkMax( right ? B : pk2( -0x8000, -0x8000 ), B2 ),
-        v[5] = pkMin( right ? C : pk2( 0x7FFF, 0x7FFF ), C2 );
+        v[3] = right ? A : pk2( 0x7FFF, 0x7FFF ), v[4] = right ? B : pk2( -0x8000, -0x8000 ), v[5] = right ? C : pk2( 0x7FFF, 0x7FFF );
 #pragma unroll
         for ( int off = 32; off > 0; off >>= 1 ) {
           v[0] = pkMin( v[0], __shfl_xor( v[0], off, 64 ) ), v[1] = pkMax( v[1], __shfl_xor( v[1], off, 64 ) ), v[2] = pkMin( v[2], __shfl_xor( v[2], off, 64 ) );
@@ -834,7 +930,6 @@
       __syncthreads();
       continue;
     }
-    if ( moved ) lvReport( next + slot + 1u, pkLo( A2 ), pkHi( A2 ), pkLo( C2 ), pkLo( A2 ), pkHi( A2 ), pkLo( C2 ) );
     if ( waveSegMinMaxPacked( key, A, B, C, lane ) )
       lvReport( next + key, pkLo( A ), pkHi( A ), pkLo( C ), pkLo( B ), pkHi( B ), ~pkHi( C ) );
   }
@@ -871,6 +966,7 @@
   __shared__ __align__( 16 ) uint32_t sWave[2][WAVES];
   __shared__ uint32_t sCount[2], sNodeBase, sDepth;
   const int      lane = threadIdx.x & 63, tid = threadIdx.x;
+  if ( a.specLevel != kNone && a.counts[a.specLevel] != 0 ) return;
   const uint32_t total = *a.retiredCount;
   const uint32_t p0    = uint32_t( tid ) * K;
   for ( uint32_t s = blockIdx.x; s < total; s += gridDim.x ) {
@@ -1202,10 +1298,12 @@
     if ( tid == 0 && sDepth ) atomicMax( a.finishDepth, sDepth );
   }
   if ( a.hostDepth && tid == 0 ) {
-    __threadfence();
+    if ( blockIdx.x < total ) __threadfence();
     if ( atomicAdd( a.ticket, 1u ) == gridDim.x - 1u ) {
       __threadfence();
       *a.hostDepth = __hip_atomic_load( a.finishDepth, __ATOMIC_RELAXED, __HIP_MEMORY_SCOPE_AGENT );
+      a.hostDepth[1] = __hip_atomic_load( a.hugeCount, __ATOMIC_RELAXED, __HIP_MEMORY_SCOPE_AGENT );
+      a.hostDepth[2] = __hip_atomic_load( a.retiredCount, __ATOMIC_RELAXED, __HIP_MEMORY_SCOPE_AGENT );
     }
   }
 }
@@ -1237,7 +1335,6 @@
   TMC2_TRY( d_work.alloc( 3 * size_t( n ) + 2 * ( size_t( tiles ) + 1 ) ) );
   TMC2_TRY( d_segs.alloc( 2 * maxSegs ) );
   TMC2_TRY( d_small.alloc( kMaxLevels + 16 ) );
-  static_assert( kMaxLevels + 16 <= 128, "lvRootKernel clears the counters with one workgroup of 128" );
   BuildArgs a;
   a.pts = d_pts, a.n = n, a.tiles = tiles, a.P = tree.ptsTree.p, a.perm = tree.perm.p;
   a.seg = d_work.p, a.loc1 = d_work.p + n, a.loc2 = d_work.p + 2 * size_t( n );
@@ -1255,6 +1352,7 @@
   a.huge         = d_huge.p;
   a.hugeCount    = d_small.p + kMaxLevels + 7;
   a.hugeMax      = hugeMax;
+  a.specLevel    = kNone;
   a.hostSmall    = nullptr;
   a.hostDepth    = ctx->answerLine( tmc2_ctx::kAnswerTreeDepth );
   a.retireMax    = uint32_t( kPieceMax );
@@ -1271,19 +1369,38 @@
   DevBuf<LvPartial> d_partial;
   const size_t     maxLv = 2 * ( size_t( n ) / ( size_t( kPieceMax ) + 1 ) + 2 );
   TMC2_TRY( d_lv.alloc( 2 * maxLv ) );
-  TMC2_TRY( d_list.alloc( size_t( tiles ) * kScanTile ) );
+  TMC2_TRY( d_list.alloc( 2 * size_t( tiles ) * kScanTile ) );
   TMC2_TRY( d_partial.alloc( size_t( n ) / ( kLandBlock * kLandRounds ) + 2 ) );
-  a.lvA = d_lv.p, a.lvB = d_lv.p + maxLv, a.list = d_list.p, a.partial = d_partial.p;
+  a.lvA = d_lv.p, a.lvB = d_lv.p + maxLv, a.list = d_list.p, a.list2 = d_list.p + size_t( tiles ) * kScanTile, a.partial = d_partial.p;
+  DevBuf<Pt>       d_P2;
+  DevBuf<uint32_t> d_perm2;
+  DevBuf<int32_t>  d_startRng;
+  const dim3       grdS( std::min<uint32_t>( grdE.x, 1024u ) );
+  TMC2_TRY( d_P2.alloc( n ) );
+  TMC2_TRY( d_perm2.alloc( n ) );
+  TMC2_TRY( d_startRng.alloc( 6 * size_t( grdS.x ) ) );
+  a.P2 = d_P2.p, a.perm2 = d_perm2.p, a.startRng = d_startRng.p;
+  if ( !ctx->kdTicket.p ) {
+    TMC2_TRY( ctx->kdTicket.alloc( 16 ) );
+    TMC2_HIP( hipMemsetAsync( ctx->kdTicket.p, 0, 64, s ) );
+    ctx->kdTickets = 0;
+  }
+  a.startTicket = ctx->kdTicket.p;
   const auto decideOpt = ctxOption( ctx, "KD_DECIDE" );
   a.decideRng = decideOpt && ( *decideOpt )[0] == 'g' ? 0u : uint32_t( kDecideRng );
-  hipLaunchKernelGGL( lvRootKernel, dim3( 1 ), dim3( 128 ), 0, s, a );
-  hipLaunchKernelGGL( lvInitKernel, dim3( std::min<uint32_t>( grdE.x, 1024u ) ), blk, 0, s, a );
-  hipLaunchKernelGGL( lvDecideKernel, dim3( 1 ), dim3( kDecideThreads ), 0, s, a, 0u );
+  hipLaunchKernelGGL( lvStartKernel, grdS, blk, 0, s, a, ctx->kdTickets );
+  ctx->kdTickets += grdS.x;
+  uint32_t ( &gridHint )[2] = ctx->kdGridHint[n >> 15].v;
+  const dim3 grdHuge( std::min<uint32_t>( gridHint[0] + gridHint[0] / 4u + 4u, 4u * uint32_t( ctx->cuCount ) ) );
+  const dim3 grdPiece( std::min<uint32_t>( gridHint[1] + gridHint[1] / 4u + 16u, 8u * uint32_t( ctx->cuCount ) ) );
+  const bool pieceProfile = bool( ctxOption( ctx, "KD_PIECE_PROFILE" ) );
   uint32_t out[kMaxLevels + 16];
   int      found = -1;
+  bool     finished = false;
   int& hint = ctx->kdLevelHint[( n >> 15 ) * 2u + 1u];
   for ( uint32_t level = 0; level < uint32_t( kMaxLevels ) && found < 0; ) {
-    uint32_t chunkEnd = level + 1;
+    uint32_t   chunkEnd    = level + 1;
+    const bool speculative = level == 0 && hint > 0 && !pieceProfile;
     if ( level == 0 && hint > 0 ) {
       chunkEnd = uint32_t( std::min( hint, kMaxLevels ) );
     } else {
@@ -1292,13 +1409,19 @@
     }
     volatile uint32_t* hostSmall = ctx->answerLine( tmc2_ctx::kAnswerTreeLevels );
     for ( ; level < chunkEnd; ++level ) {
-      hipLaunchKernelGGL( lvFlagKernel<true>, grdT, blk, 0, s, a, level );
-      hipLaunchKernelGGL( lvSwapOneKernel, grdE, blk, sumsLds, s, a, level );
-      hipLaunchKernelGGL( lvFlagKernel<false>, grdT, blk, 0, s, a, level );
-      hipLaunchKernelGGL( lvSwapTwoKernel, grdL, dim3( kLandBlock ), sumsLds, s, a, level );
+      hipLaunchKernelGGL( lvFlagKernel, grdT, blk, 0, s, a, level );
+      hipLaunchKernelGGL( lvPullOneKernel, grdT, blk, sumsLds, s, a, level );
+      hipLaunchKernelGGL( lvPullTwoKernel, grdL, dim3( kLandBlock ), sumsLds, s, a, level );
       BuildArgs ad = a;
       if ( level + 1 == chunkEnd ) ad.hostSmall = hostSmall;
       hipLaunchKernelGGL( lvDecideKernel, dim3( 1 ), dim3( kDecideThreads ), 0, s, ad, level + 1u );
+    }
+    if ( speculative ) {
+      BuildArgs as = a;
+      as.specLevel = chunkEnd;
+      TMC2_TRY( allowLargeLds( reinterpret_cast<const void*>( pieceKernel<> ), kPieceLdsBytes, ctx->device, 256 ) );
+      hipLaunchKernelGGL( hugeSegmentsKernel, grdHuge, dim3( 64 * kHugeWaves ), 0, s, as );
+      hipLaunchKernelGGL( pieceKernel<>, grdPiece, dim3( kPieceMax / kPiecePer ), kPieceLdsBytes, s, as );
     }
     TMC2_HIP( hipGetLastError() );
     TMC2_HIP( hipStreamSynchronize( s ) );
@@ -1308,6 +1431,7 @@
         found = int( l );
         break;
       }
+    finished = speculative && found >= 0;
   }
   if ( found < 0 ) {
     setError( "kdtree: more than %d levels", kMaxLevels - 1 );
@@ -1317,13 +1441,13 @@
   hint       = std::max( found, 1 );
   const int32_t* box = reinterpret_cast<const int32_t*>( out + kMaxLevels + 8 );
   for ( int d = 0; d < 3; ++d ) tree.lo[d] = box[d], tree.hi[d] = box[3 + d];
-  const uint32_t hugeSegs = out[kMaxLevels + 7];
+  const uint32_t hugeSegs = finished ? 0u : out[kMaxLevels + 7];
   if ( hugeSegs )
     hipLaunchKernelGGL( hugeSegmentsKernel, dim3( std::min<uint32_t>( hugeSegs, 4u * uint32_t( ctx->cuCount ) ) ), dim3( 64 * kHugeWaves ), 0, s, a );
-  const uint32_t retired = out[kMaxLevels + 3] + hugeSegs * ( 2u * hugeMax / uint32_t( kPieceMax ) );
+  const uint32_t retired = finished ? 0u : out[kMaxLevels + 3] + hugeSegs * ( 2u * hugeMax / uint32_t( kPieceMax ) );
   if ( retired ) {
     const dim3 grid( std::min<uint32_t>( retired, 8u * uint32_t( ctx->cuCount ) ) ), block( kPieceMax / kPiecePer );
-    if ( ctxOption( ctx, "KD_PIECE_PROFILE" ) ) {
+    if ( pieceProfile ) {
       DevBuf<unsigned long long> d_prof;
       TMC2_TRY( d_prof.alloc( 16 ) );
       TMC2_HIP( hipMemsetAsync( d_prof.p, 0, 16 * 8, s ) );
@@ -1350,6 +1474,16 @@
       return TMC2_E_UNSUPPORTED;
     }
     tree.depth = std::max( tree.depth, int( fin ) );
+    gridHint[0] = a.hostDepth[1], gridHint[1] = a.hostDepth[2];
+  }
+  if ( finished ) {
+    const uint32_t fin = *a.hostDepth;
+    if ( fin >= uint32_t( kMaxLevels ) ) {
+      setError( "kdtree: more than %d levels", kMaxLevels - 1 );
+      return TMC2_E_UNSUPPORTED;
+    }
+    tree.depth = std::max( tree.depth, int( fin ) );
+    gridHint[0] = a.hostDepth[1], gridHint[1] = a.hostDepth[2];
   }
   return TMC2_OK;
 }
```

Result: slower. 190.3 (-1.6%).
